# heyoeyo/muggled_dpt

Hardware: AMD Instinct MI355X
Metric: depth-maps/sec @518x518 (504x504 model tensor), Depth-Anything-V2 ViT-L (higher is better)
Workload: dtype bf16; 1 GPU; Depth-Anything-V2 ViT-L (vitl), 518x518 image -> 504x504 tensor, batch 32/GPU, bf16 MFMA operands + fp32 accumulate, mdpt_forward via C ABI; global_batch=32, parallelism=dp1, gemm_tile=0, batch_split=True

## Files before the change

### include/mdpt.h

```cpp
#ifndef MDPT_H
#define MDPT_H

#include <stddef.h>
#include <stdint.h>

#ifdef __cplusplus
extern "C" {
#endif

#define MDPT_ABI_VERSION 6

#define MDPT_PREC_BF16 0
#define MDPT_PREC_BF16X3 1
#define MDPT_PREC_FP16 2
#define MDPT_PREC_FP16X3 3
#define MDPT_PREC_MIXED 4

#define MDPT_CLASS_PATCH 0
#define MDPT_CLASS_QKV 1
#define MDPT_CLASS_ATTN 2
#define MDPT_CLASS_PROJ 3
#define MDPT_CLASS_FC1 4
#define MDPT_CLASS_FC2 5
#define MDPT_CLASS_REASM 6
// ... 203 lines not shown
int mdpt_post_align_metrics(const mdpt_depth_pair* pairs_host, const void* pairs_dev, int32_t P, int32_t pred_dtype, int32_t space, double tmin,
                            double tmax, const void* fit_f64, void* metrics_f64, void* scratch, size_t scratch_bytes, void* stream);
int mdpt_post_align_apply(const mdpt_depth_pair* pairs_host, const void* pairs_dev, int32_t P, int32_t pred_dtype, int32_t space, const void* fit_f64,
                          const int64_t* out_offsets_host, const void* out_offsets_dev, double dmin, double dmax, void* out_f32, void* stream);

typedef struct mdpt_guided_pair { const void* map; int32_t h, w; const void* photo; int64_t pitch; int32_t H, W; void* out; int64_t scratch_off; } mdpt_guided_pair;
int mdpt_post_guided_scratch_bytes(const mdpt_guided_pair* pairs_host, int32_t P, size_t* bytes);
int mdpt_post_guided_upsample(const mdpt_guided_pair* pairs_host, const void* pairs_dev, int32_t P, int32_t map_dtype, int32_t radius, double eps,
                              void* scratch, size_t scratch_bytes, void* coeffs_f64, void* stream);

typedef struct mdpt_texture { const void* bgr; int32_t h, w; } mdpt_texture;
int mdpt_post_render_scratch_bytes(int32_t B, int32_t V, int32_t nv, int32_t nf, int32_t out_h, int32_t out_w, size_t* bytes);
int mdpt_post_render(const void* xyz_f32, const void* uv_f32, const void* faces_i32, const void* counts_i32, int32_t B, int32_t nv, int32_t nf,
                     int32_t mode, const mdpt_texture* tex_host, const void* tex_dev, const void* view_proj_f64, int32_t V, int32_t out_h, int32_t out_w,
                     int32_t cull_back, double point_size, void* color_bgra, void* depth_f32, void* face_id_i32, void* scratch, size_t scratch_bytes,
                     void* stream);

int mdpt_post_fill_scratch_bytes(int32_t N, int32_t H, int32_t W, size_t* bytes);
int mdpt_post_fill_holes(const void* color_bgra, const void* depth_f32, int32_t N, int32_t H, int32_t W, double band, void* out_bgra, void* out_depth_f32,
                         void* scratch, size_t scratch_bytes, void* stream);

int mdpt_post_video_scratch_bytes(int32_t T, int32_t h, int32_t w, int32_t out_h, int32_t out_w, size_t* bytes);
int mdpt_post_video_fit(const void* frames, int32_t dtype, int32_t T, int32_t h, int32_t w, const void* prev_frame, const void* ab_in_f64, const void* started_i32,
                        int32_t rounds, double c, double cut_corr, void* table_f64, void* ab_out_f64, void* sums_f64, void* scratch, size_t scratch_bytes,
                        void* stream);
int mdpt_post_video_filter(const void* frames, int32_t dtype, int32_t T, int32_t h, int32_t w, const void* table_f64, const void* prev_out_f32, double alpha,
                           double tau, void* out_f32, void* stream);
int mdpt_post_video_display(const void* stable_f32, int32_t T, int32_t h, int32_t w, const void* table_f64, const void* range_in_f32, const void* started_i32,
                            int32_t out_h, int32_t out_w, int32_t reverse, const void* cmap_bgr, double range_rate, void* out_bgr, void* ranges_f32,
                            void* range_out_f32, void* scratch, size_t scratch_bytes, void* stream);

#define MDPT_REFOCUS_MAX_RADIUS 32
#define MDPT_REFOCUS_TILE 32
typedef struct mdpt_refocus_pair { const void* map; int32_t h, w; const void* photo; int64_t pitch; int32_t H, W; void* out; int64_t scratch_off, tile_off; } mdpt_refocus_pair;
int mdpt_post_refocus_scratch_bytes(const mdpt_refocus_pair* records_host, int32_t n, int32_t max_radius, size_t* bytes);
int mdpt_post_refocus(const mdpt_refocus_pair* records_host, const void* records_dev, int32_t n, int32_t dtype, int32_t space, double focus,
                      const double* focus_xy, double aperture, double focus_range, int32_t max_radius, void* scratch, size_t scratch_bytes, void* radius_out,
                      void* defocus_out, void* stream);

#define MDPT_NORMALS_MAX_STEP 16
#define MDPT_NORMALS_TILE 32
#define MDPT_NORMALS_MAX_LIGHTS 64
typedef struct mdpt_normals_pair { const void* map; int32_t h, w; const void* photo; int64_t pitch; int32_t H, W; void* normals; void* encoded; void* relit; int64_t scratch_off, tile_off; double kx, ky; int32_t step, pad; } mdpt_normals_pair;
int mdpt_post_normals_scratch_bytes(const mdpt_normals_pair* records_host, int32_t n, size_t* bytes);
int mdpt_post_normals(const mdpt_normals_pair* records_host, const void* records_dev, int32_t n, int32_t dtype, int32_t space, double min_depth,
                      double max_depth, double edge_ratio, const void* lights_dev, int32_t num_lights, double ambient, double diffuse, double specular,
                      int32_t shininess_log2, void* scratch, size_t scratch_bytes, void* stream);

#define MDPT_SHADOWS_MAX_REACH 32
#define MDPT_SHADOWS_AO_DIRECTIONS 8
typedef struct mdpt_shadows_pair { const void* map; int32_t h, w; const void* photo; int64_t pitch; int32_t H, W, gh, gw; void* ao; void* vis; void* relit; int64_t scratch_off, tile_off, gtile_off; double kx, ky; int32_t step, pad; } mdpt_shadows_pair;
int mdpt_post_shadows_scratch_bytes(const mdpt_shadows_pair* records_host, int32_t n, size_t* bytes);
int mdpt_post_shadows(const mdpt_shadows_pair* records_host, const void* records_dev, int32_t n, int32_t dtype, int32_t space, double min_depth,
                      double max_depth, double edge_ratio, const void* lights_dev, int32_t num_lights, double ambient, double diffuse, double specular,
                      int32_t shininess_log2, int32_t shadow_reach, double shadow_bias, double shadow_thickness, int32_t ao_reach, double ao_radius,
                      double ao_bias, double ao_strength, void* scratch, size_t scratch_bytes, void* stream);

#define MDPT_SEGMENT_TILE 32
typedef struct mdpt_segment_image { const void* map; int32_t h, w; void* labels; int64_t scratch_off, region_off, tile_off, pixel_off; } mdpt_segment_image;
typedef struct mdpt_segment_photo { const void* labels; int32_t h, w; const void* photo; int64_t pitch; int32_t H, W; void* bgra; void* mask; int64_t region_off; int32_t regions, pad; } mdpt_segment_photo;
int mdpt_segment_scratch_bytes(const mdpt_segment_image* records_host, int32_t n, size_t* bytes);
int mdpt_segment_depth(const mdpt_segment_image* records_host, const void* records_dev, int32_t n, int32_t dtype, int32_t space, double step,
                       int32_t connectivity, int32_t min_area, void* scratch, size_t scratch_bytes, void* counts, void* area, void* bbox, void* first,
                       void* vrange, void* sum_q, void* range, void* stream);
int mdpt_segment_colors(const mdpt_segment_image* records_host, const void* records_dev, int32_t n, void* colors, void* stream);
int mdpt_segment_cutout(const mdpt_segment_photo* records_host, const void* records_dev, int32_t n, const void* picks_dev, int32_t num_picks,
                        int32_t by_label, void* selected, size_t selected_bytes, int32_t invert, void* stream);

#define MDPT_LOCALFIT_MAX_GRID 256
#define MDPT_LOCALFIT_MAX_RADIUS 64
#define MDPT_LOCALFIT_CHUNK 2048
typedef struct mdpt_localfit_pair { const void* pred; int32_t ph, pw; const void* truth; const void* valid; int32_t H, W, gh, gw; int64_t cell_off, scratch_off; void* out; } mdpt_localfit_pair;
int mdpt_localfit_scratch_bytes(const mdpt_localfit_pair* records_host, int32_t n, size_t* bytes);
int mdpt_localfit_fit(const mdpt_localfit_pair* records_host, const void* records_dev, int32_t n, int32_t pred_dtype, int32_t space, int32_t radius,
                      double prior, double tmin, double tmax, void* moments_f64, void* fit_f64, void* sums_f64, void* coeffs_f64, void* scratch,
                      size_t scratch_bytes, void* stream);
int mdpt_localfit_apply(const mdpt_localfit_pair* records_host, const void* records_dev, int32_t n, int32_t pred_dtype, int32_t space,
                        const void* coeffs_f64, double dmin, double dmax, void* stream);

int mdpt_export_tap(mdpt_handle* h, int32_t which, void* out_f32, void* workspace, size_t workspace_bytes, void* stream);

int mdpt_debug_set_stop(mdpt_handle* h, int32_t block, int32_t step);
int mdpt_debug_set_ksplit_min(mdpt_handle* h, int32_t min_k_tiles, int32_t four_k_tiles);
int mdpt_debug_set_reassemble_overlap(mdpt_handle* h, int32_t on);
int mdpt_debug_set_wscale_policy(mdpt_handle* h, int32_t all);
int mdpt_debug_set_side_stream_priority(mdpt_handle* h, int32_t prio);
int mdpt_debug_set_side_stream_probe(mdpt_handle* h, int32_t on);
int mdpt_debug_side_stream_info(mdpt_handle* h, int32_t* candidates, int32_t* rejected);
int mdpt_debug_read(mdpt_handle* h, const char* name, void* out_f32, size_t out_floats, void* workspace, size_t workspace_bytes,
                    void* stream);

int mdpt_debug_set_operand_format(int32_t fp16);

int mdpt_debug_gemm(const void* a_bf16, const void* w_bf16, void* out_f32, void* out_bf16, int32_t M, int32_t N, int32_t K,
                    int32_t tile, int32_t iters, void* stream, void* dbg_times_or_null);
int mdpt_debug_attention(const void* q_bf16, const void* k_bf16, const void* vt_bf16, void* out_bf16, int32_t B, int32_t heads, int32_t N,
                         int32_t npad, int32_t npadv, int32_t iters, void* stream);
typedef struct mdpt_attn_form {
    const void* q_hi; const void* q_lo; const void* k_hi; const void* k_lo;
    const void* vt_hi; const void* vt_lo;
    void* out_hi; void* out_lo;
    int32_t B, heads, N, npad, npadv, F;
    int32_t x3;
    const float* bias_lut; int32_t bias_elen; const int32_t* tq; const int32_t* tk;
    int32_t head_dim;
    int32_t win_nw; const int32_t* rowmap; const int32_t* region; int32_t region_ld;
    int32_t bias_run4;
    int32_t bias_row;
    int32_t bias_ww;
    const float* swin_ls;
    int32_t out_ld;
    int32_t allow_split_kv;
} mdpt_attn_form;
int mdpt_debug_attention_form(const mdpt_attn_form* form, void* stream);
int mdpt_debug_attn_weights_form(const mdpt_attn_form* form, void* out_f32, void* stream);
int mdpt_debug_conv3(const void* in_bf16, const void* w_packed_bf16, const void* bias_f32, const void* skip_f32, const void* up_f32, int32_t Hu,
                     int32_t Wu, void* out_f32, void* out_bf16, int32_t relu_bf16, int32_t B, int32_t H, int32_t W, int32_t Cin, int32_t Cout,
                     int32_t path, int32_t tile, int32_t iters, void* stream, void* dbg_times, const void* in_lo_bf16_or_null,
                     const void* w_lo_bf16_or_null, void* out_lo_bf16_or_null);
typedef struct mdpt_gemm_form {
    const void* a_hi; const void* a_lo; const void* w_hi; const void* w_lo;
    int32_t M, N, K, lda, ldw, npass;
    int32_t amode, ekind, tile, act;
    int32_t tok_np, tok_stride;
    int32_t Hi, Wi, Cin, Ho, Wo, cstride;
    const void* bias; const void* gamma; const void* resid;
    int32_t ldr, bias_img_stride, bias_img_rows;
    void* out_f32; void* out_hi; void* out_lo;
    int32_t ldc, relu_bf16, acc_init;
    const void* wscale;
    void* q_hi; void* q_lo; void* k_hi; void* k_lo; void* vt_hi; void* vt_lo;
    int32_t F, heads, npad, npadv;
    float qscale;
    const void* pos;
    int32_t d2s_k, d2s_cout;
    const void* head_w; const void* head_b; void* head_out;
    int32_t head_sigmoid, head_out_dtype;
    int32_t ksplit, ks_all;
    void* ks_part;
} mdpt_gemm_form;
int mdpt_debug_gemm_form(const mdpt_gemm_form* form, void* stream);
int mdpt_debug_ksplit_finish(const mdpt_gemm_form* form, void* stream);

int mdpt_profile_enable(int on);
int mdpt_profile_report(char* json_buf, size_t capacity);

int mdpt_set_gemm_tile(mdpt_handle* h, int32_t tile);

int mdpt_allgather(void* comm, const void* send_dev, void* recv_dev, size_t count_per_rank, int32_t dtype, void* stream);

#ifdef __cplusplus
}
#endif
#endif
```

### muggled_dpt_amd/csrc/gemm.hip

```cpp

#include "mdpt_kernels.h"
#include "mdpt_prof.h"
#include "f8_cross.h"
#include <stdio.h>
#include <stdlib.h>

#pragma clang fp contract(off)

namespace {

#include "mfma_common.inc"
#include "gemm_common.inc"
#include "gemm_epilogue_strip.inc"
#include "gemm_lockstep.inc"
#include "gemm8_epilogues.inc"
#include "gemm8.inc"

template <int AMODE, int EKIND, int DMODE, bool F8 = false>
int launch_pp_mode(const GemmParams& p, hipStream_t stream) {
    constexpr unsigned LDS = 2 * 65536;
    if constexpr (MDPT_OP_IS_F16 && !F8 && (EKIND == MDPT_E_GENERIC || EKIND == MDPT_E_D2S) && DMODE != DM_RINIT) {
        if (p.f8) return launch_pp_mode<AMODE, EKIND, DMODE, true>(p, stream);
    }
    constexpr auto kern = gemm8_kernel<AMODE, EKIND, DMODE, F8>;
    if (const int e = mdpt_lds_limit<kern>(LDS)) return e;
    const int tiles = ((p.M + 255) / 256) * ((p.N + 255) / 256);
    const char* prof_name = mdpt_kernel_label<kern>(F8 ? "gemm8_kernel<%d, %d, %d, f8>" : "gemm8_kernel<%d, %d, %d>", AMODE, EKIND, DMODE);
    MdptProfScope prof(prof_name, 2.0 * (p.M_alg > 0 ? p.M_alg : p.M) * p.N * p.K, stream);
    const int ks = (AMODE == MDPT_A_DENSE && EKIND == MDPT_E_GENERIC && DMODE == DM_F32 && p.ksplit > 1) ? p.ksplit : 1;
    hipLaunchKernelGGL(kern, dim3(tiles, ks), dim3(512), LDS, stream, p);
    return (int)hipGetLastError();
}

template <int AMODE, int EKIND>
int launch_pp(const GemmParams& p, hipStream_t stream) {
    if constexpr (EKIND == MDPT_E_GENERIC) {
        const int dmode = generic_direct_mode(p);
        if (dmode == DM_BF16) return launch_pp_mode<AMODE, EKIND, DM_BF16>(p, stream);
        if (dmode == DM_RESID) return launch_pp_mode<AMODE, EKIND, DM_RESID>(p, stream);
        if (dmode == DM_F32) return launch_pp_mode<AMODE, EKIND, DM_F32>(p, stream);
        if constexpr (AMODE == MDPT_A_DENSE) {
            if (dmode == DM_RINIT) return launch_pp_mode<AMODE, EKIND, DM_RINIT>(p, stream);
        }
        return launch_pp_mode<AMODE, EKIND, DM_NONE>(p, stream);
    } else if constexpr (EKIND == MDPT_E_QKV) {
        return launch_pp_mode<AMODE, EKIND, DM_QK>(p, stream);
    } else if constexpr (EKIND == MDPT_E_SWQKV) {
        return launch_pp_mode<AMODE, EKIND, DM_SWQK>(p, stream);
    } else {
        return launch_pp_mode<AMODE, EKIND, DM_NONE>(p, stream);
    }
}

template <int BM, int BN, int WM, int WN, int BK, int NST, int MINW, int AMODE, int EKIND, bool F8 = false>
int launch_cfg(const GemmParams& p, hipStream_t stream) {
    constexpr int LDS = NST * (BM + BN) * BK * 2;
    if constexpr (MDPT_OP_IS_F16 && !F8 && BK == 64 && (EKIND == MDPT_E_GENERIC || EKIND == MDPT_E_D2S) && !(BM == 256 && BN == 256)) {
        if (p.f8) return launch_cfg<BM, BN, WM, WN, BK, NST, MINW, AMODE, EKIND, true>(p, stream);
    }
    constexpr auto kern = gemm_kernel<BM, BN, WM, WN, BK, NST, MINW, AMODE, EKIND, F8>;
    if (const int e = mdpt_lds_limit<kern>(LDS)) return e;
    const int tiles = ((p.M + BM - 1) / BM) * ((p.N + BN - 1) / BN);
    const char* prof_name = mdpt_kernel_label<kern>(F8 ? "gemm_kernel<%d, %d, %d, %d, %d, %d, %d, %d, %d, f8>" : "gemm_kernel<%d, %d, %d, %d, %d, %d, %d, %d, %d>", BM, BN, WM, WN, BK, NST, MINW, AMODE, EKIND);
    MdptProfScope prof(prof_name, 2.0 * (p.M_alg > 0 ? p.M_alg : p.M) * p.N * p.K, stream);
    const int ks = ((AMODE == MDPT_A_DENSE || AMODE == MDPT_A_CONV3) && EKIND == MDPT_E_GENERIC && BM == 64 && BN == 64 && BK == 64 && p.ksplit > 1) ? p.ksplit : 1;
    hipLaunchKernelGGL(kern, dim3(tiles, ks), dim3(64 * WM * WN), LDS, stream, p);
    return (int)hipGetLastError();
}

int resolve_tile(const GemmParams& p) {
    int tile = p.tile;
    if (p.ksplit > 1 && p.ks_all) return MDPT_TILE_64x64;
    if (p.ksplit > 1) {
        const long wgs = (long)((p.M + 255) / 256) * ((p.N + 255) / 256) * p.ksplit;
        const int kt = (p.K / 64 / p.ksplit) * p.npass;
        const bool pp = p.tile == MDPT_TILE_PP256 || (p.tile == MDPT_TILE_AUTO && wgs >= (p.throughput_mode ? 70 : 140));
        return (pp && p.amode == MDPT_A_DENSE && generic_direct_mode(p) == DM_F32 && kt >= 4 && !(kt & 1) && (p.N & 255) == 0) ? MDPT_TILE_PP256 : MDPT_TILE_64x64;
    }
    if (tile == MDPT_TILE_AUTO) {
        const long tiles256 = (long)((p.M + 255) / 256) * ((p.N + 255) / 256);
        const long tiles128 = (long)((p.M + 127) / 128) * ((p.N + 127) / 128);
        const long ncol = (p.N + 255) / 256 * 256;
        const bool cols_ok = (ncol - p.N) * 4 <= ncol;
        const bool big = cols_ok && tiles256 >= (p.throughput_mode ? 70 : 140);
        tile = big ? MDPT_TILE_PP256 : (tiles128 <= 352 ? MDPT_TILE_64x64 : MDPT_TILE_128x128);
        if (!big && tiles128 > 352 && p.N <= 64) return -1;
    }
    if (tile == MDPT_TILE_PP256 && (((p.K / 64) * p.npass) & 1) && !p.f8) tile = (p.K / 64) * p.npass <= 3 && p.tile == MDPT_TILE_AUTO ? MDPT_TILE_64x64 : MDPT_TILE_256x256;
    if (tile == MDPT_TILE_PP256 && p.f8 && ((p.K & 255) || (p.N & 255))) tile = MDPT_TILE_128x128;
    if (tile == MDPT_TILE_256x256 && p.f8) tile = MDPT_TILE_128x128;
    if (tile == MDPT_TILE_PP256 && p.bias_img_stride && p.ekind == MDPT_E_QKV && !(HAVE_IMGB && p.bias_img_rows >= 256)) tile = MDPT_TILE_256x256;
    return tile;
}
template <int AMODE, int EKIND>
int launch_tile(const GemmParams& p, hipStream_t stream) {
    int tile = resolve_tile(p);
    if (tile < 0) return launch_cfg<128, 64, 4, 1, 64, 2, 2, AMODE, EKIND>(p, stream);
    if constexpr (EKIND == MDPT_E_GENERIC) {
        if (tile == MDPT_TILE_PP256 && p.acc_init &&
            !(AMODE == MDPT_A_DENSE && generic_direct_mode(p) == DM_RINIT && (p.K / 64) * p.npass >= 4 && !p.f8))
            tile = MDPT_TILE_256x256;
    }
    if (tile == MDPT_TILE_64x64) {
        if constexpr ((AMODE == MDPT_A_DENSE || AMODE == MDPT_A_CONV3) && EKIND == MDPT_E_GENERIC) {
            if (ktiles_total(p, p.K / (p.ksplit > 1 ? p.ksplit : 1)) >= 32) return launch_cfg<64, 64, 2, 2, 64, 3, 1, AMODE, EKIND>(p, stream);
        }
        return launch_cfg<64, 64, 2, 2, 64, 2, 1, AMODE, EKIND>(p, stream);
    }
    if (tile == MDPT_TILE_PP256) return launch_pp<AMODE, EKIND>(p, stream);
    if (tile == MDPT_TILE_256x128) return launch_cfg<256, 128, 2, 2, 32, 3, 2, AMODE, EKIND>(p, stream);
    if (tile == MDPT_TILE_256x256) return launch_cfg<256, 256, 2, 4, 64, 2, 1, AMODE, EKIND>(p, stream);
    return launch_cfg<128, 128, 2, 2, 64, 2, 1, AMODE, EKIND>(p, stream);
}
// ... 51 lines not shown
```

### muggled_dpt_amd/csrc/gemm8.inc

```
template <int AMODE, bool F8 = false>
struct HalfStager {
    static constexpr int A_BYTES = 256 * 128;
#ifdef MDPT_GEMM8_BUF_STAGING
    static constexpr bool BUFFERED = AMODE != MDPT_A_CONV3;
#else
    static constexpr bool BUFFERED = false;
#endif
    __amdgpu_buffer_rsrc_t rs_a, rs_w;
    unsigned a_voff[4], b_voff;
    int a_soff, b_soff, a_row_step, b_row_step;
    const op_t* a_base_hi; const op_t* a_base_lo; const op_t* w_base_hi; const op_t* w_base_lo;
    size_t a_bytes, w_bytes;
    const op_t* a_ptr[4];
    int a_pix[4], a_y[4], a_x[4], a_ko[4];
    const op_t* b_ptr[4];
    ptrdiff_t a_hi_minus_lo, w_lo_minus_hi;
    const op_t* conv_plane;
    int a_pass, a_k0, a_tap, a_ci, b_pass, b_k0;
    int st_m0, st_n0, b_step;
    bool a_f8, b_f8;

    __device__ __forceinline__ void place_a(const GemmParams& p, int pass, int wave, int lane) {
        const int lrow = lane >> 3;
        a_f8 = pass < p.npass - 1;
// ... 128 lines not shown
                const size_t e = (size_t)(a_pix[i] + iy * p.Wi + ix) * p.Cin + a_ci;
                src = ok ? conv_plane + ((F8 && a_f8) ? (e >> 1) : e) + a_ko[i] : p.zero_page + a_ko[i];
            } else {
                src = a_ptr[i];
                a_ptr[i] += 64;
            }
            glds16(src, buf + (wave + 8 * i) * 1024);
        }
        if (F8 && H == 1 && a_f8) {
            a_k0 += 128;
            if (AMODE == MDPT_A_CONV3) { if (++a_tap == 9) { a_tap = 0; a_ci += 128; } }
            if (a_k0 == p.K) {
                a_k0 = 0; a_tap = 0; a_ci = 0;
                ++a_pass;
                place_a(p, a_pass, wave, threadIdx.x & 63);
            }
        } else
        if (H == 1) {
            a_k0 += 64;
            if (AMODE == MDPT_A_CONV3) {
                if (++a_tap == 9) { a_tap = 0; a_ci += 64; }
            }
            if (a_k0 == p.K) {
                a_k0 = 0; a_tap = 0; a_ci = 0;
                const ptrdiff_t da = (a_pass == 0 ? a_hi_minus_lo : 0) - p.K;
                if (a_pass == 0) conv_plane = p.A_hi;
#pragma unroll
                for (int i = 0; i < 4; ++i)
                    if (AMODE != MDPT_A_CONV3) a_ptr[i] += da;
                ++a_pass;
            }
        }
    }

    template <int H>
    __device__ __forceinline__ void issue_b(const GemmParams& p, char* buf, int wave) {
        typedef __attribute__((address_space(3))) void* lds_ptr_t;
        if constexpr (BUFFERED) {
#pragma unroll
            for (int i = 2 * H; i < 2 * H + 2; ++i)
                __builtin_amdgcn_raw_ptr_buffer_load_lds(rs_w, (lds_ptr_t)(buf + A_BYTES + (wave + 8 * i) * 1024), 16, b_voff, b_soff + i * b_row_step, 0, 0);
            if (H == 1) {
                b_soff += 128;
                if (b_soff == p.K * 2) {
                    b_soff = 0;
                    rs_w = rsrc(b_pass == 0 ? w_base_lo : w_base_hi, w_bytes);
                    ++b_pass;
                }
            }
            return;
        }
        if constexpr (F8) {
#pragma unroll
            for (int i = 2 * H; i < 2 * H + 2; ++i) glds16((const op_t*)((const char*)b_ptr[0] + i * b_step), buf + A_BYTES + (wave + 8 * i) * 1024);
            if (H == 1) b_ptr[0] += 64;
        } else {
#pragma unroll
        for (int i = 2 * H; i < 2 * H + 2; ++i) {
            glds16(b_ptr[i], buf + A_BYTES + (wave + 8 * i) * 1024);
            b_ptr[i] += 64;
        }
        }
        if (F8 && H == 1 && b_f8) {
            b_k0 += 128;
            if (b_k0 == p.K) {
                b_k0 = 0;
                ++b_pass;
                place_b(p, b_pass, wave, threadIdx.x & 63);
            }
        } else
        if (H == 1) {
            b_k0 += 64;
            if (b_k0 == p.K) {
                b_k0 = 0;
                const ptrdiff_t dw = (b_pass == 0 ? w_lo_minus_hi : -w_lo_minus_hi) - p.K;
#pragma unroll
                for (int i = 0; i < 4; ++i) b_ptr[i] += dw;
                ++b_pass;
            }
        }
    }
};

template <int AMODE, int EKIND, bool SW, bool RI = false, bool FAST = false, bool F8 = false>
__device__ __forceinline__ void gemm8_body(const GemmParams& p, char* smem, const int dmode, const int m0, const int n0,
                                           const unsigned long long t_start) {
    static_assert(!RI || SW, "residual-initialised accumulators use the swapped operand order (4 consecutive columns per lane)");
    static_assert(!F8 || (!FAST && !RI && MDPT_HAVE_F8), "fp8 cross terms: state-machine stager, fp16 build");
    static_assert(!FAST || AMODE == MDPT_A_DENSE, "the stateless staging is for dense rows");
    constexpr int A_BYTES = 256 * 128, BUF = 2 * A_BYTES;
    const int tid = threadIdx.x, lane = tid & 63;
    const int wave = __builtin_amdgcn_readfirstlane(tid >> 6);
    const int grp = wave >> 2, wc = wave & 3;
    unsigned long long t_first = 0, t_loop = 0;
    constexpr bool swapped = SW;
    HalfStager<AMODE, F8> st;
    if constexpr (!FAST) st.init(p, m0, n0, wave, lane);
    typedef __attribute__((address_space(3))) void* lds_ptr_t;
    __amdgpu_buffer_rsrc_t rs_a, rs_w;
    unsigned fa_voff = 0, fb_voff = 0;
    int fa_step = 0, fb_step = 0;
    if constexpr (FAST) {
        const int rows_here = p.M - m0 < 256 ? p.M - m0 : 256, cols_here = p.N - n0 < 256 ? p.N - n0 : 256;
        rs_a = tile_rsrc(p.A_hi + (size_t)m0 * p.lda, (size_t)rows_here * p.lda * 2);
        rs_w = tile_rsrc(p.W_hi + (size_t)n0 * p.ldw, ((size_t)(cols_here - 1) * p.ldw + p.K) * 2);
        const int r = wave * 8 + (lane >> 3);
        const int koff = ((lane & 7) ^ ((r >> 1) & 7)) * 8;
        fa_voff = (unsigned)(r * p.lda + koff) * 2u;
        fb_voff = (unsigned)(r * p.ldw + koff) * 2u;
        fa_step = 64 * p.lda * 2;
        fb_step = 64 * p.ldw * 2;
    }
#define ISSUE_A(H_, BUF_, KB_)                                                                                          \
    do {                                                                                                                \
        if constexpr (FAST) {                                                                                           \
            _Pragma("unroll") for (int i = 2 * (H_); i < 2 * (H_) + 2; ++i)                                             \
                __builtin_amdgcn_raw_ptr_buffer_load_lds(rs_a, (lds_ptr_t)((BUF_) + (wave + 8 * i) * 1024), 16, fa_voff, (KB_) + i * fa_step, 0, 0); \
        } else {                                                                                                        \
            st.template issue_a<H_>(p, BUF_, wave);                                                                     \
        }                                                                                                               \
    } while (0)
#define ISSUE_B(H_, BUF_, KB_)                                                                                          \
    do {                                                                                                                \
        if constexpr (FAST) {                                                                                           \
            _Pragma("unroll") for (int i = 2 * (H_); i < 2 * (H_) + 2; ++i)                                             \
                __builtin_amdgcn_raw_ptr_buffer_load_lds(rs_w, (lds_ptr_t)((BUF_) + 256 * 128 + (wave + 8 * i) * 1024), 16, fb_voff, (KB_) + i * fb_step, 0, 0); \
        } else {                                                                                                        \
            st.template issue_b<H_>(p, BUF_, wave);                                                                     \
        }                                                                                                               \
    } while (0)

    const int l15 = lane & 15, lh = lane >> 4, key = (l15 >> 1) & 7;
    const int a_off0 = (grp * 64 + l15) * 128 + ((lh ^ key) << 4), a_off1 = (grp * 64 + l15) * 128 + (((4 + lh) ^ key) << 4);
    const int b_off0 = A_BYTES + (wc * 32 + l15) * 128 + ((lh ^ key) << 4), b_off1 = A_BYTES + (wc * 32 + l15) * 128 + (((4 + lh) ^ key) << 4);

    f32x4 acc[2][2][4][2];
    if constexpr (!RI) {
#pragma unroll
        for (int a = 0; a < 2; ++a)
#pragma unroll
            for (int b = 0; b < 2; ++b)
#pragma unroll
                for (int i = 0; i < 4; ++i)
#pragma unroll
                    for (int j = 0; j < 2; ++j) acc[a][b][i][j] = f32x4{0.0f, 0.0f, 0.0f, 0.0f};
    }

    opx8 fa[4][2], fb0[2][2], fb1[2][2];
#define LOAD_A(QM_, BUF_)                                                                                             \
    do {                                                                                                              \
        _Pragma("unroll") for (int i = 0; i < 4; ++i) {                                                               \
            fa[i][0] = *(const opx8*)(smem + (BUF_) * BUF + (QM_) * 16384 + i * 2048 + a_off0);                      \
            fa[i][1] = *(const opx8*)(smem + (BUF_) * BUF + (QM_) * 16384 + i * 2048 + a_off1);                      \
        }                                                                                                             \
    } while (0)
#define LOAD_B(DST_, QN_, BUF_)                                                                                       \
    do {                                                                                                              \
        _Pragma("unroll") for (int j = 0; j < 2; ++j) {                                                               \
            DST_[j][0] = *(const opx8*)(smem + (BUF_) * BUF + (QN_) * 16384 + j * 2048 + b_off0);                    \
            DST_[j][1] = *(const opx8*)(smem + (BUF_) * BUF + (QN_) * 16384 + j * 2048 + b_off1);                    \
        }                                                                                                             \
    } while (0)
#define MFMA_Q(QM_, QN_, FB_)                                                                                         \
    do {                                                                                                              \
        __builtin_amdgcn_s_setprio(1);                                                                                \
        _Pragma("unroll") for (int kk = 0; kk < 2; ++kk)                                                              \
            _Pragma("unroll") for (int i = 0; i < 4; ++i)                                                             \
                _Pragma("unroll") for (int j = 0; j < 2; ++j)                                                         \
                    acc[QM_][QN_][i][j] = swapped ? MDPT_MFMA_16x16x32(FB_[j][kk], fa[i][kk], acc[QM_][QN_][i][j], 0, 0, 0) \
                                                  : MDPT_MFMA_16x16x32(fa[i][kk], FB_[j][kk], acc[QM_][QN_][i][j], 0, 0, 0); \
        __builtin_amdgcn_s_setprio(0);                                                                                \
    } while (0)
#if MDPT_HAVE_F8
    int wsc = 0, wsc_lo = 0;
    const int asc = F8_A_SCALE;
    if constexpr (F8) {
#pragma unroll
        for (int b4 = 0; b4 < 4; ++b4) {
            int n = n0 + (b4 >> 1) * 128 + wc * 32 + (b4 & 1) * 16 + l15;
            n = n < p.N ? n : p.N - 1;
            wsc |= (int)p.S8[n] << (8 * b4);
            if (p.npass == 3) wsc_lo |= (int)p.S8_lo[n] << (8 * b4);
        }
    }
#define MFMA_Q8_ONE(QM_, QN_, FB_, I_, J_, WS_)                                                                       \
    do {                                                                                                              \
        if constexpr (swapped) f8_mfma16_w_first<2 * (QN_) + (J_)>(acc[QM_][QN_][I_][J_], f8_cat(FB_[J_][0], FB_[J_][1]), f8_cat(fa[I_][0], fa[I_][1]), WS_, asc); \
        else f8_mfma16_a_first<2 * (QN_) + (J_)>(acc[QM_][QN_][I_][J_], f8_cat(fa[I_][0], fa[I_][1]), f8_cat(FB_[J_][0], FB_[J_][1]), asc, WS_); \
    } while (0)
#define MFMA_Q8(QM_, QN_, FB_, WS_)                                                                                   \
    do {                                                                                                              \
        __builtin_amdgcn_s_setprio(1);                                                                                \
        MFMA_Q8_ONE(QM_, QN_, FB_, 0, 0, WS_); MFMA_Q8_ONE(QM_, QN_, FB_, 0, 1, WS_);                                 \
        MFMA_Q8_ONE(QM_, QN_, FB_, 1, 0, WS_); MFMA_Q8_ONE(QM_, QN_, FB_, 1, 1, WS_);                                 \
        MFMA_Q8_ONE(QM_, QN_, FB_, 2, 0, WS_); MFMA_Q8_ONE(QM_, QN_, FB_, 2, 1, WS_);                                 \
        MFMA_Q8_ONE(QM_, QN_, FB_, 3, 0, WS_); MFMA_Q8_ONE(QM_, QN_, FB_, 3, 1, WS_);                                 \
        __builtin_amdgcn_s_setprio(0);                                                                                \
    } while (0)
#endif
#define ACC_READY(QM_, QN_, N_)                                                                                                          \
    asm volatile("s_waitcnt vmcnt(" #N_ ")"                                                                                              \
                 : "+v"(acc[QM_][QN_][0][0]), "+v"(acc[QM_][QN_][0][1]), "+v"(acc[QM_][QN_][1][0]), "+v"(acc[QM_][QN_][1][1]),           \
                   "+v"(acc[QM_][QN_][2][0]), "+v"(acc[QM_][QN_][2][1]), "+v"(acc[QM_][QN_][3][0]), "+v"(acc[QM_][QN_][3][1])            \
                 :                                                                                                                       \
                 : "memory")

    const int T = F8 ? ktiles_total(p, p.K) : (p.K / 64) * p.npass;
    const int T8 = F8 ? ktiles_f8(p, p.K) : 0, T8a = F8 ? p.K / 128 : 0;
    char* const bufE = smem;
    char* const bufO = smem + BUF;
    ISSUE_A(0, bufE, 0);
    ISSUE_B(0, bufE, 0);
    ISSUE_B(1, bufE, 0);
    ISSUE_A(1, bufE, 0);
    if constexpr (RI) {
        constexpr unsigned OOB = 0xFFFFFFF0u;
        typedef __attribute__((ext_vector_type(4))) int i32x4;
        const int rows_here = p.M - m0 < 256 ? p.M - m0 : 256;
        const unsigned long long base = (unsigned long long)(p.resid + (size_t)m0 * p.ldr);
        i32x4 rs;
        rs[0] = __builtin_amdgcn_readfirstlane((int)(unsigned)base);
        rs[1] = __builtin_amdgcn_readfirstlane((int)(unsigned)(base >> 32) & 0xFFFF);
        rs[2] = __builtin_amdgcn_readfirstlane((int)(unsigned)((size_t)rows_here * p.ldr * 4));
        rs[3] = 0x00020000;
        const unsigned row_b = (unsigned)p.ldr * 4u;
        auto load_quadrant = [&](int qm, int qn) {
#pragma unroll
            for (int j = 0; j < 2; ++j) {
                const int nc = n0 + qn * 128 + wc * 32 + j * 16 + 4 * lh;
                const unsigned col = nc < p.N ? (unsigned)nc * 4u : OOB;
#pragma unroll
                for (int i = 0; i < 4; ++i) {
                    const unsigned row = (unsigned)(qm * 128 + grp * 64 + i * 16 + l15) * row_b;
                    const unsigned off = col == OOB ? OOB : row + col;
                    asm volatile("s_nop 4\n\tbuffer_load_dwordx4 %0, %1, %2, 0 offen" : "=v"(acc[qm][qn][i][j]) : "v"(off), "s"(rs) : "memory");
                }
            }
        };
        load_quadrant(0, 0);
        ISSUE_B(0, bufO, 128);
        ISSUE_A(0, bufO, 128);
        ISSUE_B(1, bufO, 128);
        ISSUE_A(1, bufO, 128);
        load_quadrant(0, 1);
        load_quadrant(1, 1);
        load_quadrant(1, 0);
        WAIT_VM(40);
    } else {
        ISSUE_B(0, bufO, 128);
        ISSUE_A(0, bufO, 128);
        ISSUE_B(1, bufO, 128);
        ISSUE_A(1, bufO, 128);
        WAIT_VM(8);
    }
    BAR();
    if (p.dbg_times) t_first = memtime_now();
    if (grp == 1) BAR();


    const float ri_scale = (MDPT_OP_IS_F16 && RI && p.wscale) ? p.wscale[0] : 1.0f;
#define SCALE_Q(QM_, QN_)                                                                                             \
    do {                                                                                                              \
        if (MDPT_OP_IS_F16 && RI && ri_scale != 1.0f) {                                                               \
            _Pragma("unroll") for (int i = 0; i < 4; ++i)                                                             \
                _Pragma("unroll") for (int j = 0; j < 2; ++j) acc[QM_][QN_][i][j] *= ri_scale;                        \
        }                                                                                                             \
    } while (0)
#define GEMM8_ITER(MORE_, FIRST_, MQ)                                                                                       \
    do {                                                                                                              \
        const int kE = t * 128 + 256, kO = kE + 128;         \
                                                                                                              \
        LOAD_B(fb0, 0, 0); PIN(); LOAD_A(0, 0); PIN();                                                                \
        WAIT_LGKM(8); BAR(); WAIT_LGKM(0); PIN();                                                                     \
        if (FIRST_) { ACC_READY(0, 0, 32); SCALE_Q(0, 0); PIN(); }                     \
        MQ(0, 0, fb0); BAR();                                                                                     \
                                                                                                              \
        LOAD_B(fb1, 1, 0); PIN();                                                                                     \
        if (MORE_) ISSUE_B(0, bufE, kE);                                                             \
        BAR(); WAIT_LGKM(0); PIN();                                                                                   \
        if (FIRST_) { ACC_READY(0, 1, 18); SCALE_Q(0, 1); PIN(); }                               \
        MQ(0, 1, fb1); BAR();                                                                                     \
                                                                                                              \
        LOAD_A(1, 0); PIN();                                                                                          \
        if (MORE_) ISSUE_A(0, bufE, kE);                                                             \
        PIN(); WAIT_LGKM(0); BAR(); PIN();                                                                            \
        if (FIRST_) { ACC_READY(1, 1, 12); SCALE_Q(1, 1); PIN(); }                                \
        MQ(1, 1, fb1); BAR();                                                                                     \
                                                                                                              \
        if (MORE_) { ISSUE_B(1, bufE, kE); ISSUE_A(1, bufE, kE); PIN(); WAIT_VM(8); } else { WAIT_VM(0); }                      \
        BAR();                                                                                                        \
        if (FIRST_) { ACC_READY(1, 0, 8); SCALE_Q(1, 0); PIN(); }  \
        MQ(1, 0, fb0); BAR();                                                                                     \
                                                                                                              \
        LOAD_B(fb0, 0, 1); PIN(); LOAD_A(0, 1); PIN();                                                                \
        WAIT_LGKM(8); BAR(); WAIT_LGKM(0); PIN();                                                                     \
        MQ(0, 0, fb0); BAR();                                                                                     \
                                                                                                              \
        LOAD_B(fb1, 1, 1); PIN();                                                                                     \
        if (MORE_) ISSUE_B(0, bufO, kO);                                                             \
        BAR(); WAIT_LGKM(0); PIN();                                                                                   \
        MQ(0, 1, fb1); BAR();                                                                                     \
                                                                                                              \
        LOAD_A(1, 1); PIN();                                                                                          \
        if (MORE_) ISSUE_A(0, bufO, kO);                                                             \
        PIN(); WAIT_LGKM(0); BAR(); PIN();                                                                            \
        MQ(1, 1, fb1); BAR();                                                                                     \
                                                                                                              \
        if (MORE_) { ISSUE_B(1, bufO, kO); ISSUE_A(1, bufO, kO); PIN(); WAIT_VM(8); }                                          \
        BAR();                                                                                                        \
        MQ(1, 0, fb0); BAR();                                                                                     \
    } while (0)
    if constexpr (FAST) {
        int t = 0;
        if constexpr (RI) {
            GEMM8_ITER(true, true, MFMA_Q);
            t = 2;
        }
        for (; t + 2 < T; t += 2) GEMM8_ITER(true, false, MFMA_Q);
        GEMM8_ITER(false, false, MFMA_Q);
    } else {
        int t = 0;
#if MDPT_HAVE_F8
        if constexpr (F8) {
#define MQ8A(QM_, QN_, FB_) MFMA_Q8(QM_, QN_, FB_, wsc)
#define MQ8B(QM_, QN_, FB_) MFMA_Q8(QM_, QN_, FB_, wsc_lo)
            for (; t < T8a; t += 2) GEMM8_ITER(true, false, MQ8A);
            for (; t < T8; t += 2) GEMM8_ITER(true, false, MQ8B);
#undef MQ8A
#undef MQ8B
        }
#endif
        for (; t < T; t += 2) {
            const bool more = t + 2 < T;
            GEMM8_ITER(more, (RI && t == 0), MFMA_Q);
        }
    }
#undef GEMM8_ITER
#undef SCALE_Q
#undef ACC_READY
#undef ISSUE_A
#undef ISSUE_B
    if (grp == 0) BAR();
#undef LOAD_A
#undef LOAD_B
#undef MFMA_Q
#if MDPT_HAVE_F8
#undef MFMA_Q8
#undef MFMA_Q8_ONE
#endif
    if (p.dbg_times) t_loop = memtime_now();
    if constexpr (SW) {
        if (EKIND == MDPT_E_SWQKV) {
            if (dmode == DM_F32) {
                if (HAVE_IMGB && p.bias_img_stride) epilogue_direct<DM_F32, false, MDPT_ACT_NONE, HAVE_IMGB>(p, acc, m0, n0, grp, wc, lane);
                else epilogue_direct<DM_F32, false, MDPT_ACT_NONE>(p, acc, m0, n0, grp, wc, lane);
            } else if (HAVE_IMGB && p.bias_img_stride) {
                if (p.q_lo) epilogue_swin_qk<true, HAVE_IMGB>(p, acc, m0, n0, grp, wc, lane);
                else epilogue_swin_qk<false, HAVE_IMGB>(p, acc, m0, n0, grp, wc, lane);
            } else if (p.q_lo) {
                epilogue_swin_qk<true>(p, acc, m0, n0, grp, wc, lane);
            } else {
                epilogue_swin_qk<false>(p, acc, m0, n0, grp, wc, lane);
            }
        } else if (EKIND == MDPT_E_QKV) {
            if (HAVE_IMGB && p.bias_img_stride) {
                if (p.q_lo) epilogue_direct<DM_QK, true, MDPT_ACT_NONE, HAVE_IMGB>(p, acc, m0, n0, grp, wc, lane);
                else epilogue_direct<DM_QK, false, MDPT_ACT_NONE, HAVE_IMGB>(p, acc, m0, n0, grp, wc, lane);
            } else if (p.q_lo) epilogue_direct<DM_QK, true, MDPT_ACT_NONE>(p, acc, m0, n0, grp, wc, lane);
            else epilogue_direct<DM_QK, false, MDPT_ACT_NONE>(p, acc, m0, n0, grp, wc, lane);
        } else if (HAVE_IMGB && dmode == DM_BF16 && p.bias_img_stride) {
            if (p.act == MDPT_ACT_GELU) {
                if (p.out_lo) epilogue_direct<DM_BF16, true, MDPT_ACT_GELU, HAVE_IMGB>(p, acc, m0, n0, grp, wc, lane);
                else epilogue_direct<DM_BF16, false, MDPT_ACT_GELU, HAVE_IMGB>(p, acc, m0, n0, grp, wc, lane);
            } else {
                if (p.out_lo) epilogue_direct<DM_BF16, true, MDPT_ACT_NONE, HAVE_IMGB>(p, acc, m0, n0, grp, wc, lane);
                else epilogue_direct<DM_BF16, false, MDPT_ACT_NONE, HAVE_IMGB>(p, acc, m0, n0, grp, wc, lane);
            }
        } else if (dmode == DM_BF16) {
            const int sel = (p.out_lo ? 3 : 0) + (p.act == MDPT_ACT_GELU ? 2 : (p.act == MDPT_ACT_RELU || p.relu_bf16) ? 1 : 0);
            switch (sel) {
                case 0: epilogue_direct<DM_BF16, false, MDPT_ACT_NONE>(p, acc, m0, n0, grp, wc, lane); break;
                case 1: epilogue_direct<DM_BF16, false, MDPT_ACT_RELU>(p, acc, m0, n0, grp, wc, lane); break;
                case 2: epilogue_direct<DM_BF16, false, MDPT_ACT_GELU>(p, acc, m0, n0, grp, wc, lane); break;
                case 3: epilogue_direct<DM_BF16, true, MDPT_ACT_NONE>(p, acc, m0, n0, grp, wc, lane); break;
                case 4: epilogue_direct<DM_BF16, true, MDPT_ACT_RELU>(p, acc, m0, n0, grp, wc, lane); break;
                default: epilogue_direct<DM_BF16, true, MDPT_ACT_GELU>(p, acc, m0, n0, grp, wc, lane); break;
            }
        } else if (dmode == DM_F32 || dmode == DM_RINIT) {
            if (HAVE_IMGB && p.bias_img_stride) epilogue_direct<DM_F32, false, MDPT_ACT_NONE, HAVE_IMGB>(p, acc, m0, n0, grp, wc, lane);
            else epilogue_direct<DM_F32, false, MDPT_ACT_NONE>(p, acc, m0, n0, grp, wc, lane);
        } else {
            epilogue_direct<DM_RESID, false, MDPT_ACT_NONE>(p, acc, m0, n0, grp, wc, lane);
        }
        if (p.dbg_times && tid == 0) {
            const unsigned long long t_issued = memtime_now();
            stamp_record(p.dbg_times, t_start, t_first, t_loop, STAMP_HW_ID, t_issued);
        }
        return;
    }
    if ((EKIND == MDPT_E_QKV && dmode == DM_VT) || (EKIND == MDPT_E_SWQKV && dmode == DM_SWVT)) {
        if (EKIND == MDPT_E_SWQKV) {
            if (HAVE_IMGB && p.bias_img_stride) {
                if (p.vt_lo) epilogue_swin_vt<true, HAVE_IMGB>(p, acc, m0, n0, grp, wc, lane);
                else epilogue_swin_vt<false, HAVE_IMGB>(p, acc, m0, n0, grp, wc, lane);
            } else if (p.vt_lo) epilogue_swin_vt<true>(p, acc, m0, n0, grp, wc, lane);
            else epilogue_swin_vt<false>(p, acc, m0, n0, grp, wc, lane);
        } else if (HAVE_IMGB && p.bias_img_stride) {
            if (p.vt_lo) epilogue_direct_vt<true, HAVE_IMGB>(p, acc, m0, n0, grp, wc, lane);
            else epilogue_direct_vt<false, HAVE_IMGB>(p, acc, m0, n0, grp, wc, lane);
        } else if (p.vt_lo) {
            epilogue_direct_vt<true>(p, acc, m0, n0, grp, wc, lane);
        } else {
            epilogue_direct_vt<false>(p, acc, m0, n0, grp, wc, lane);
        }
        if (p.dbg_times && tid == 0) stamp_record(p.dbg_times, t_start, t_first, t_loop, STAMP_NO_ID);
        return;
    }
    __syncthreads();

    float* strip = (float*)smem + wave * (32 * 32);
#pragma unroll
    for (int qm = 0; qm < 2; ++qm)
#pragma unroll
        for (int qn = 0; qn < 2; ++qn)
#pragma unroll
            for (int rb = 0; rb < 2; ++rb) {
#pragma unroll
                for (int ii = 0; ii < 2; ++ii)
#pragma unroll
                    for (int j = 0; j < 2; ++j)
#pragma unroll
                        for (int r = 0; r < 4; ++r) strip[(ii * 16 + 4 * lh + r) * 32 + j * 16 + l15] = acc[qm][qn][rb * 2 + ii][j][r];
                epilogue_block<32, EKIND>(p, strip, lane, m0 + qm * 128 + grp * 64 + rb * 32, n0 + qn * 128 + wc * 32);
            }
    if (p.dbg_times && tid == 0) stamp_record(p.dbg_times, t_start, t_first, t_loop, 4);
}

__host__ __device__ inline int generic_direct_mode(const GemmParams& p) {
    const bool imgb_ok = HAVE_IMGB && p.bias_img_rows >= 256 && p.bias && !p.gamma && !p.relu_bf16 && p.act != MDPT_ACT_RELU;
    const bool plain = !p.up_src && (!p.bias_img_stride || imgb_ok);
    const bool fits = (size_t)256 * p.ldc * 4 < 0xFFFFFFF0ull;
    if (plain && fits && p.out_hi && !p.out_f32 && !p.gamma && !p.resid && !(p.relu_bf16 && p.act != MDPT_ACT_NONE)) return DM_BF16;
    if (plain && fits && !p.bias_img_stride && p.out_f32 && !p.out_hi && p.gamma && p.resid && p.resid == p.out_f32 && p.bias && p.act == MDPT_ACT_NONE && p.ldr == p.ldc)
        return DM_RESID;
    if (plain && fits && p.acc_init && p.out_f32 && !p.out_hi && !p.gamma && p.resid == p.out_f32 && p.ldr == p.ldc && p.act == MDPT_ACT_NONE && !p.relu_bf16)
        return DM_RINIT;
    if (plain && fits && p.out_f32 && !p.out_hi && !p.gamma && !p.resid && p.act == MDPT_ACT_NONE && !p.relu_bf16) return DM_F32;
    return DM_NONE;
}

template <int AMODE, int EKIND, int DMODE, bool F8 = false>
__global__ __launch_bounds__(512, 1) void gemm8_kernel(const GemmParams p) {
    extern __shared__ __attribute__((aligned(16))) char smem[];
    unsigned long long t_start = 0;
    if (p.dbg_times) t_start = memtime_now();
    int m0, n0;
    tile_coords((p.N + 255) / 256, 256, 256, m0, n0);
    if constexpr (EKIND == MDPT_E_SWQKV) {
        const bool fast = p.npass == 1;
        if (n0 >= 2 * p.F && p.swin_vtokmap) {
            if (fast) gemm8_body<AMODE, EKIND, false, false, true>(p, smem, DM_SWVT, m0, n0, t_start);
            else gemm8_body<AMODE, EKIND, false>(p, smem, DM_SWVT, m0, n0, t_start);
        } else {
            const int dm = n0 >= 2 * p.F ? DM_F32 : DM_SWQK;
            if (fast) gemm8_body<AMODE, EKIND, true, false, true>(p, smem, dm, m0, n0, t_start);
            else gemm8_body<AMODE, EKIND, true>(p, smem, dm, m0, n0, t_start);
        }
    } else if (EKIND == MDPT_E_QKV) {
#ifdef MDPT_GEMM8_NO_FAST
        const bool fast = false;
#else
        const bool fast = AMODE == MDPT_A_DENSE && p.npass == 1;
#endif
        if (n0 + 256 <= 2 * p.F && (size_t)p.M * p.F * 2 < 0xFFFFFFF0ull) {
            if constexpr (AMODE == MDPT_A_DENSE) {
                if (fast) gemm8_body<AMODE, EKIND, true, false, true>(p, smem, DM_QK, m0, n0, t_start);
                else gemm8_body<AMODE, EKIND, true>(p, smem, DM_QK, m0, n0, t_start);
            } else {
                gemm8_body<AMODE, EKIND, true>(p, smem, DM_QK, m0, n0, t_start);
            }
        } else if (n0 >= 2 * p.F && n0 + 256 <= p.N && (size_t)(p.M / p.npad) * p.F * p.npadv * 2 < 0xFFFFFFF0ull) {
            if constexpr (AMODE == MDPT_A_DENSE) {
                if (fast) gemm8_body<AMODE, EKIND, false, false, true>(p, smem, DM_VT, m0, n0, t_start);
                else gemm8_body<AMODE, EKIND, false>(p, smem, DM_VT, m0, n0, t_start);
            } else {
                gemm8_body<AMODE, EKIND, false>(p, smem, DM_VT, m0, n0, t_start);
            }
        } else {
            gemm8_body<AMODE, EKIND, false>(p, smem, DM_NONE, m0, n0, t_start);
        }
    } else if constexpr (AMODE == MDPT_A_DENSE && DMODE == DM_F32) {
        if constexpr (F8) {
            gemm8_body<AMODE, EKIND, true, false, false, true>(p, smem, DMODE, m0, n0, t_start);
            return;
        }
        GemmParams q = p;
        if (p.ksplit > 1) {
            const int z = (int)blockIdx.y, ks = p.K / p.ksplit;
            q.K = ks;
            q.A_hi = p.A_hi + z * ks; q.W_hi = p.W_hi + z * ks;
            if (p.npass >= 2) q.A_lo = p.A_lo + z * ks;
            if (p.npass == 3) q.W_lo = p.W_lo + z * ks;
            if (z > 0) { q.bias = nullptr; q.bias_img_stride = 0; q.out_f32 = p.ks_part + (size_t)(z - 1) * p.M * p.ldc; }
        }
        if (q.npass == 1) gemm8_body<AMODE, EKIND, true, false, true>(q, smem, DMODE, m0, n0, t_start);
        else gemm8_body<AMODE, EKIND, true, false, false>(q, smem, DMODE, m0, n0, t_start);
    } else if constexpr (AMODE == MDPT_A_DENSE && DMODE != DM_NONE) {
#ifdef MDPT_GEMM8_NO_FAST
        if (false) {}
#else
        if (p.npass == 1) gemm8_body<AMODE, EKIND, true, DMODE == DM_RINIT, true>(p, smem, DMODE, m0, n0, t_start);
#endif
        else if constexpr (F8) gemm8_body<AMODE, EKIND, true, false, false, true>(p, smem, DMODE, m0, n0, t_start);
        else gemm8_body<AMODE, EKIND, true, DMODE == DM_RINIT, false>(p, smem, DMODE, m0, n0, t_start);
    } else {
        if constexpr (F8) gemm8_body<AMODE, EKIND, DMODE != DM_NONE, false, false, true>(p, smem, DMODE, m0, n0, t_start);
        else gemm8_body<AMODE, EKIND, DMODE != DM_NONE, DMODE == DM_RINIT>(p, smem, DMODE, m0, n0, t_start);
    }
}
```

### muggled_dpt_amd/csrc/gemm8_epilogues.inc

```
constexpr bool HAVE_IMGB = MDPT_OP_IS_F16 != 0;
enum { DM_NONE = 0, DM_BF16 = 1, DM_RESID = 2, DM_QK = 3, DM_VT = 4, DM_F32 = 5, DM_RINIT = 6, DM_SWQK = 7, DM_SWVT = 8 };

__device__ __forceinline__ __amdgpu_buffer_rsrc_t tile_rsrc(const void* base, size_t bytes) {
    return __builtin_amdgcn_make_buffer_rsrc(const_cast<void*>(base), 0, (int)(unsigned)(bytes < 0xFFFFFFF0ull ? bytes : 0xFFFFFFF0ull), 0x00020000);
}

template <int MODE, bool X3, int ACT, bool IMGB = false>
__device__ __forceinline__ void epilogue_direct(const GemmParams& p, f32x4 (&acc)[2][2][4][2], int m0, int n0, int grp, int wc, int lane) {
    constexpr unsigned OOB = 0xFFFFFFF0u;
    const int l15 = lane & 15, lh = lane >> 4;
    const int rows_here = p.M - m0 < 256 ? p.M - m0 : 256;
    int bnd = 1 << 30;
    const float* bias0 = p.bias;
    const float* bias1 = p.bias;
    if (IMGB) {
        const int img0 = m0 / p.bias_img_rows;
        bnd = (img0 + 1) * p.bias_img_rows - m0;
        bias0 = p.bias + (size_t)img0 * p.bias_img_stride;
        bias1 = bnd < rows_here ? bias0 + p.bias_img_stride : bias0;
    }
    auto pick = [&](const f32x4& a, const f32x4& b, bool next) {
        f32x4 r;
#pragma unroll
        for (int e = 0; e < 4; ++e) r[e] = next ? b[e] : a[e];
        return r;
    };

    if (MODE == DM_F32) {
        const __amdgpu_buffer_rsrc_t rs = tile_rsrc(p.out_f32 + (size_t)m0 * p.ldc, (size_t)rows_here * p.ldc * 4);
        const unsigned row_b = (unsigned)p.ldc * 4u;
        const float inv_s = (MDPT_OP_IS_F16 && p.wscale) ? p.wscale[1] : 1.0f;
#pragma unroll
        for (int qn = 0; qn < 2; ++qn) {
            f32x4 bias[2], biasn[2];
            unsigned col_off[2];
#pragma unroll
            for (int j = 0; j < 2; ++j) {
                const int nc = n0 + qn * 128 + wc * 32 + j * 16 + 4 * lh;
                bias[j] = p.bias ? *(const f32x4*)(bias0 + (nc < p.N ? nc : p.N - 4)) : f32x4{0.0f, 0.0f, 0.0f, 0.0f};
                if (IMGB) biasn[j] = *(const f32x4*)(bias1 + (nc < p.N ? nc : p.N - 4));
                col_off[j] = nc < p.N ? (unsigned)nc * 4u : OOB;
            }
#pragma unroll
            for (int qm = 0; qm < 2; ++qm)
#pragma unroll
                for (int i = 0; i < 4; ++i) {
                    const unsigned row = (unsigned)(qm * 128 + grp * 64 + i * 16 + l15) * row_b;
                    const bool next = IMGB && qm * 128 + grp * 64 + i * 16 + l15 >= bnd;
#pragma unroll
                    for (int j = 0; j < 2; ++j) {
                        const f32x4 a = MDPT_OP_IS_F16 ? acc[qm][qn][i][j] * inv_s : acc[qm][qn][i][j];
                        const f32x4 v = a + (IMGB ? pick(bias[j], biasn[j], next) : bias[j]);
                        __builtin_amdgcn_raw_buffer_store_b128(__builtin_bit_cast(u32x4, v), rs, col_off[j] == OOB ? OOB : row + col_off[j], 0, 0);
                    }
                }
        }
        return;
    }
    if (MODE == DM_RESID) {
        const __amdgpu_buffer_rsrc_t rs = tile_rsrc(p.out_f32 + (size_t)m0 * p.ldc, (size_t)rows_here * p.ldc * 4);
        const unsigned row_b = (unsigned)p.ldc * 4u;
        f32x4 bias[2][2], gam[2][2];
        unsigned col_off[2][2];
#pragma unroll
        for (int qn = 0; qn < 2; ++qn)
#pragma unroll
            for (int j = 0; j < 2; ++j) {
                const int nc = n0 + qn * 128 + wc * 32 + j * 16 + 4 * lh;
                const int ncl = nc < p.N ? nc : p.N - 4;
                bias[qn][j] = *(const f32x4*)(p.bias + ncl);
                gam[qn][j] = *(const f32x4*)(p.gamma + ncl);
                col_off[qn][j] = nc < p.N ? (unsigned)nc * 4u : OOB;
            }
        auto row_off = [&](int g, int i) { return (unsigned)((g >> 1) * 128 + grp * 64 + i * 16 + l15) * row_b; };
        u32x4 old[4][4][2];
        f32x4 res[2][4][2];
        auto load_group = [&](int g) {
#pragma unroll
            for (int i = 0; i < 4; ++i)
#pragma unroll
                for (int j = 0; j < 2; ++j) {
                    const unsigned c = col_off[g & 1][j];
                    old[g][i][j] = __builtin_amdgcn_raw_buffer_load_b128(rs, c == OOB ? OOB : row_off(g, i) + c, 0, 0);
                }
        };
        auto value = [&](int g, int i, int j) {
            return (acc[g >> 1][g & 1][i][j] + bias[g & 1][j]) * gam[g & 1][j] + __builtin_bit_cast(f32x4, old[g][i][j]);
        };
        auto store = [&](int g, int i, int j, f32x4 v) {
            const unsigned c = col_off[g & 1][j];
            __builtin_amdgcn_raw_buffer_store_b128(__builtin_bit_cast(u32x4, v), rs, c == OOB ? OOB : row_off(g, i) + c, 0, 0);
        };
        unsigned long long* stamp = p.dbg_times && threadIdx.x == 0 ? p.dbg_times + (size_t)gridDim.x * 6 + (size_t)blockIdx.x * 16 : nullptr;
        if (stamp) stamp[0] = memtime_now();
        load_group(0);
        load_group(1);
        if (p.dbg_times) {
            if (stamp) stamp[1] = memtime_now();
            asm volatile("s_waitcnt vmcnt(0)" ::: "memory");
            if (stamp) stamp[2] = memtime_now();
        }
#pragma unroll
        for (int g = 0; g < 2; ++g)
#pragma unroll
            for (int i = 0; i < 4; ++i)
#pragma unroll
                for (int j = 0; j < 2; ++j) res[g][i][j] = value(g, i, j);
        load_group(2);
        load_group(3);
#pragma unroll
        for (int g = 0; g < 2; ++g)
#pragma unroll
            for (int i = 0; i < 4; ++i)
#pragma unroll
                for (int j = 0; j < 2; ++j) store(g, i, j, res[g][i][j]);
        if (p.dbg_times) {
            if (stamp) stamp[3] = memtime_now();
            asm volatile("s_waitcnt vmcnt(16)" ::: "memory");
            if (stamp) stamp[4] = memtime_now();
        }
#pragma unroll
        for (int g = 2; g < 4; ++g)
#pragma unroll
            for (int i = 0; i < 4; ++i)
#pragma unroll
                for (int j = 0; j < 2; ++j) store(g, i, j, value(g, i, j));
        if (stamp) stamp[5] = memtime_now();
        return;
    }

    __amdgpu_buffer_rsrc_t rs_hi, rs_lo;
    __amdgpu_buffer_rsrc_t rs_lo8 = tile_rsrc(p.out_hi, 0), rs_a8 = rs_lo8;
    if (MODE == DM_BF16) {
        rs_hi = tile_rsrc(p.out_hi + (size_t)m0 * p.ldc, (size_t)rows_here * p.ldc * 2);
        rs_lo = tile_rsrc(X3 ? p.out_lo + (size_t)m0 * p.ldc : p.out_hi, X3 ? (size_t)rows_here * p.ldc * 2 : 0);
        if (MDPT_HAVE_F8 && X3 && p.out_f8) {
            rs_lo8 = tile_rsrc((const unsigned char*)p.out_lo + (size_t)m0 * p.ldc, (size_t)rows_here * p.ldc);
            rs_a8 = tile_rsrc((const unsigned char*)p.out_lo + p.out_f8 + (size_t)m0 * p.ldc, p.out_a8 ? (size_t)rows_here * p.ldc : 0);
        }
    }
    f32x4 bias_q[2][2], biasn_q[2][2], gam_q[2][2];
#pragma unroll
    for (int qn = 0; qn < 2; ++qn)
#pragma unroll
        for (int j = 0; j < 2; ++j) {
            const int ncol = n0 + qn * 128 + wc * 32 + j * 16 + 4 * lh;
            const int nc = ncol < p.N ? ncol : p.N - 4;
            bias_q[qn][j] = p.bias ? *(const f32x4*)(bias0 + nc) : f32x4{0.0f, 0.0f, 0.0f, 0.0f};
            if (IMGB) biasn_q[qn][j] = *(const f32x4*)(bias1 + nc);
            if (MODE == DM_QK && ncol < p.F) gam_q[qn][j] = f32x4{p.qscale, p.qscale, p.qscale, p.qscale};
            else if (MODE == DM_QK) gam_q[qn][j] = f32x4{1.0f, 1.0f, 1.0f, 1.0f};
        }
#pragma unroll
    for (int qn = 0; qn < 2; ++qn) {
        const int nq = n0 + qn * 128 + wc * 32;
        const int n8 = nq + (lh & 1) * 16 + (lh >> 1) * 8;
        const f32x4(&bias)[2] = bias_q[qn];
        const f32x4(&biasn)[2] = biasn_q[qn];
        const f32x4(&gam)[2] = gam_q[qn];
        int qk_h = 0, qk_d = 0;
        if (MODE == DM_QK) {
            const int which = __builtin_amdgcn_readfirstlane(nq >= p.F);
            const int fcol = n8 - which * p.F;
            qk_h = fcol >> 6; qk_d = fcol & 63;
            const size_t plane = (size_t)p.M * p.F * 2;
            rs_hi = tile_rsrc(which ? p.k_hi : p.q_hi, plane);
            rs_lo = tile_rsrc(X3 ? (which ? p.k_lo : p.q_lo) : p.q_hi, X3 ? plane : 0);
        }
        const bool nok = n8 < p.N;
#pragma unroll
        for (int qm = 0; qm < 2; ++qm) {
            const int rfirst = qm * 128 + grp * 64 + l15;
            int qb = 0, qt = 0;
            if (MODE == DM_QK) {
                qb = (m0 + rfirst) / p.npad;
                qt = m0 + rfirst - qb * p.npad;
            }
#pragma unroll
            for (int i = 0; i < 4; ++i) {
                f32x4 v[2];
                const bool next = IMGB && rfirst + 16 * i >= bnd;
#pragma unroll
                for (int j = 0; j < 2; ++j) {
                    v[j] = acc[qm][qn][i][j] + (IMGB ? pick(bias[j], biasn[j], next) : bias[j]);
                    if (MODE == DM_QK) {
                        v[j] *= gam[j];
                    } else if (ACT == MDPT_ACT_GELU) {
#pragma unroll
                        for (int e = 0; e < 4; e += 2) {
                            const gelu_f32x2 g2 = gelu_erf2(gelu_f32x2{v[j][e], v[j][e + 1]});
                            v[j][e] = g2[0];
                            v[j][e + 1] = g2[1];
                        }
                    } else if (ACT == MDPT_ACT_RELU) {
#pragma unroll
                        for (int e = 0; e < 4; ++e) v[j][e] = fmaxf(v[j][e], 0.0f);
                    }
                }
                unsigned hw_[2][2], lw_[2][2];
#pragma unroll
                for (int j = 0; j < 2; ++j)
#pragma unroll
                    for (int w2 = 0; w2 < 2; ++w2) {
                        const f32x2 pp = {v[j][2 * w2], v[j][2 * w2 + 1]};
                        const opx2 hh = to_op2(pp);
                        hw_[j][w2] = __builtin_bit_cast(unsigned, hh);
                        if (X3) {
                            const f32x2 rr = pp - __builtin_convertvector(hh, f32x2);
                            lw_[j][w2] = __builtin_bit_cast(unsigned, to_op2(rr));
                        }
                    }
                unsigned ph[4], pl[4];
#pragma unroll
                for (int w2 = 0; w2 < 2; ++w2) {
                    auto r = __builtin_amdgcn_permlane16_swap(hw_[0][w2], hw_[1][w2], false, false);
                    ph[w2] = r[0];
                    ph[w2 + 2] = r[1];
                    if (X3) {
                        auto rl = __builtin_amdgcn_permlane16_swap(lw_[0][w2], lw_[1][w2], false, false);
                        pl[w2] = rl[0];
                        pl[w2 + 2] = rl[1];
                    }
                }
                unsigned off;
                if (MODE == DM_BF16) {
                    off = ((unsigned)(rfirst + 16 * i) * (unsigned)p.ldc + (unsigned)n8) * 2u;
                    if (!nok) off = OOB;
                } else {
                    off = (unsigned)((((size_t)(qb * p.heads + qk_h) * p.npad + qt) * 64 + qk_d) * 2);
                    if (!nok || m0 + rfirst + 16 * i >= p.M) off = OOB;
                }
                __builtin_amdgcn_raw_buffer_store_b128(u32x4{ph[0], ph[1], ph[2], ph[3]}, rs_hi, off, 0, 0);
#if MDPT_HAVE_F8
                if (X3 && MODE == DM_BF16 && p.out_f8) {
                    float hv[2][4], vv[2][4];
// ... 131 lines not shown
                    auto r = __builtin_amdgcn_permlane16_swap(hw_[0][w2], hw_[1][w2], false, false);
                    ph[w2] = r[0];
                    ph[w2 + 2] = r[1];
                    if (X3) {
                        auto rl = __builtin_amdgcn_permlane16_swap(lw_[0][w2], lw_[1][w2], false, false);
                        pl[w2] = rl[0];
                        pl[w2 + 2] = rl[1];
                    }
                }
                const unsigned off = dst[qm][i] < 0 ? OOB : (unsigned)(((size_t)(dst[qm][i] + hrow) * 32 + d8) * 2);
                __builtin_amdgcn_raw_buffer_store_b128(u32x4{ph[0], ph[1], ph[2], ph[3]}, rs_hi, off, 0, 0);
                if (X3) __builtin_amdgcn_raw_buffer_store_b128(u32x4{pl[0], pl[1], pl[2], pl[3]}, rs_lo, off, 0, 0);
            }
    }
}

template <bool X3, bool IMGB = false>
__device__ __forceinline__ void epilogue_swin_vt(const GemmParams& p, f32x4 (&acc)[2][2][4][2], int m0, int n0, int grp, int wc, int lane) {
    constexpr unsigned OOB = 0xFFFFFFF0u;
    const int l15 = lane & 15, lh = lane >> 4;
    const size_t plane = (size_t)(p.M / p.swin_N) * p.swin_img_velems * 2;
    const __amdgpu_buffer_rsrc_t rs_hi = tile_rsrc(p.vt_hi, plane);
    const __amdgpu_buffer_rsrc_t rs_lo = tile_rsrc(X3 ? p.vt_lo : p.vt_hi, X3 ? plane : 0);
    int bnd = 1 << 30;
    const float* bias0 = p.bias;
    const float* bias1 = p.bias;
    if (IMGB) {
        const int rows_here = p.M - m0 < 256 ? p.M - m0 : 256;
        const int img0 = m0 / p.bias_img_rows;
        bnd = (img0 + 1) * p.bias_img_rows - m0;
        bias0 = p.bias + (size_t)img0 * p.bias_img_stride;
        bias1 = bnd < rows_here ? bias0 + p.bias_img_stride : bias0;
    }
    float bias_q[2][2], biasn_q[2][2];
    int col_q[2][2];
#pragma unroll
    for (int qn = 0; qn < 2; ++qn)
#pragma unroll
        for (int j = 0; j < 2; ++j) {
            const int n = n0 + qn * 128 + wc * 32 + j * 16 + l15;
            bias_q[qn][j] = p.bias ? bias0[n < p.N ? n : p.N - 1] : 0.0f;
            if (IMGB) biasn_q[qn][j] = bias1[n < p.N ? n : p.N - 1];
            col_q[qn][j] = n < p.N ? (n - 2 * p.F) * p.npadv : -1;
        }
    int dst[2][4];
#pragma unroll
    for (int qm = 0; qm < 2; ++qm) {
        const int r0 = m0 + qm * 128 + grp * 64 + 4 * lh;
        int img = r0 / p.swin_N, t = r0 - img * p.swin_N;
#pragma unroll
        for (int i = 0; i < 4; ++i) {
            dst[qm][i] = r0 + 16 * i < p.M ? img * p.swin_img_velems + p.swin_vtokmap[t] : -1;
            t += 16;
            while (t >= p.swin_N) { t -= p.swin_N; ++img; }
        }
    }
#pragma unroll
    for (int qn = 0; qn < 2; ++qn)
#pragma unroll
        for (int qm = 0; qm < 2; ++qm)
#pragma unroll
            for (int i = 0; i < 4; ++i)
#pragma unroll
                for (int j = 0; j < 2; ++j) {
                    const bool next = IMGB && qm * 128 + grp * 64 + 16 * i + 4 * lh >= bnd;
                    const f32x4 v = acc[qm][qn][i][j] + (next ? biasn_q[qn][j] : bias_q[qn][j]);
                    unsigned hw_[2], lw_[2];
#pragma unroll
                    for (int w2 = 0; w2 < 2; ++w2) {
                        const f32x2 pp = {v[2 * w2], v[2 * w2 + 1]};
                        const opx2 hb = to_op2(pp);
                        hw_[w2] = __builtin_bit_cast(unsigned, hb);
                        if (X3) {
                            const f32x2 rr = pp - __builtin_convertvector(hb, f32x2);
                            lw_[w2] = __builtin_bit_cast(unsigned, to_op2(rr));
                        }
                    }
                    const unsigned off = dst[qm][i] < 0 || col_q[qn][j] < 0 ? OOB : (unsigned)(dst[qm][i] + col_q[qn][j]) * 2u;
                    __builtin_amdgcn_raw_buffer_store_b64(u32x2{hw_[0], hw_[1]}, rs_hi, off, 0, 0);
                    if (X3) __builtin_amdgcn_raw_buffer_store_b64(u32x2{lw_[0], lw_[1]}, rs_lo, off, 0, 0);
                }
}

template <bool X3, bool IMGB = false>
__device__ __forceinline__ void epilogue_direct_vt(const GemmParams& p, f32x4 (&acc)[2][2][4][2], int m0, int n0, int grp, int wc, int lane) {
    constexpr unsigned OOB = 0xFFFFFFF0u;
    const int l15 = lane & 15, lh = lane >> 4;
    const size_t plane = (size_t)(p.M / p.npad) * p.F * p.npadv * 2;
    const __amdgpu_buffer_rsrc_t rs_hi = tile_rsrc(p.vt_hi, plane);
    const __amdgpu_buffer_rsrc_t rs_lo = tile_rsrc(X3 ? p.vt_lo : p.vt_hi, X3 ? plane : 0);
    int bnd = 1 << 30;
    const float* bias0 = p.bias;
    const float* bias1 = p.bias;
    if (IMGB) {
        const int rows_here = p.M - m0 < 256 ? p.M - m0 : 256;
        const int img0 = m0 / p.bias_img_rows;
        bnd = (img0 + 1) * p.bias_img_rows - m0;
        bias0 = p.bias + (size_t)img0 * p.bias_img_stride;
        bias1 = bnd < rows_here ? bias0 + p.bias_img_stride : bias0;
    }
    float bias_q[2][2], biasn_q[2][2];
#pragma unroll
    for (int qn = 0; qn < 2; ++qn)
#pragma unroll
        for (int j = 0; j < 2; ++j) {
            const int n = n0 + qn * 128 + wc * 32 + j * 16 + l15;
            bias_q[qn][j] = bias0[n < p.N ? n : p.N - 1];
            if (IMGB) biasn_q[qn][j] = bias1[n < p.N ? n : p.N - 1];
        }
#pragma unroll
    for (int qn = 0; qn < 2; ++qn) {
        const int ncol = n0 + qn * 128 + wc * 32 + (lh & 1) * 16 + l15;
        const int fcol = ncol - 2 * p.F, hh = fcol >> 6, dd = fcol & 63;
        const bool nok = ncol < p.N;
#pragma unroll
        for (int qm = 0; qm < 2; ++qm) {
            const int mfirst = m0 + qm * 128 + grp * 64 + (lh >> 1) * 8;
            int qb = mfirst / p.npad, qt = mfirst - qb * p.npad;
#pragma unroll
            for (int i = 0; i < 4; ++i) {
                unsigned hw_[2][2], lw_[2][2];
#pragma unroll
                for (int j = 0; j < 2; ++j) {
                    const bool next = IMGB && qm * 128 + grp * 64 + 16 * i + 4 * lh >= bnd;
                    const f32x4 v = acc[qm][qn][i][j] + (next ? biasn_q[qn][j] : bias_q[qn][j]);
#pragma unroll
                    for (int w2 = 0; w2 < 2; ++w2) {
                        const f32x2 pp = {v[2 * w2], v[2 * w2 + 1]};
                        const opx2 hb = to_op2(pp);
                        hw_[j][w2] = __builtin_bit_cast(unsigned, hb);
                        if (X3) {
                            const f32x2 rr = pp - __builtin_convertvector(hb, f32x2);
                            lw_[j][w2] = __builtin_bit_cast(unsigned, to_op2(rr));
                        }
                    }
                }
                unsigned ph[4], pl[4];
#pragma unroll
                for (int w2 = 0; w2 < 2; ++w2) {
                    auto r = __builtin_amdgcn_permlane16_swap(hw_[0][w2], hw_[1][w2], false, false);
                    ph[w2] = r[0];
                    ph[w2 + 2] = r[1];
                    if (X3) {
                        auto rl = __builtin_amdgcn_permlane16_swap(lw_[0][w2], lw_[1][w2], false, false);
                        pl[w2] = rl[0];
                        pl[w2 + 2] = rl[1];
                    }
                }
                unsigned off = (unsigned)((((size_t)(qb * p.heads + hh) * 64 + dd) * p.npadv + qt) * 2);
                if (!nok || mfirst + 16 * i >= p.M) off = OOB;
                __builtin_amdgcn_raw_buffer_store_b128(u32x4{ph[0], ph[1], ph[2], ph[3]}, rs_hi, off, 0, 0);
                if (X3) __builtin_amdgcn_raw_buffer_store_b128(u32x4{pl[0], pl[1], pl[2], pl[3]}, rs_lo, off, 0, 0);
                qt += 16;
                while (qt >= p.npad) { qt -= p.npad; ++qb; }
            }
        }
    }
}
```

### muggled_dpt_amd/csrc/gemm_common.inc

```
#define MDPT_GELU_Q0 1.1511051654815674f
#define MDPT_GELU_Q1 0.4592081904411316f
#define MDPT_GELU_Q2 0.052496179938316345f
#define MDPT_GELU_Q3 -0.00706342002376914f
#define MDPT_GELU_Q4 0.00013693643268197775f
#define MDPT_GELU_Q5 0.00018618021567817777f
#define MDPT_GELU_Q6 -3.93776863347739e-05f
#define MDPT_GELU_Q7 2.8349124931992264e-06f
__device__ __forceinline__ float gelu_erf(float v) {
    const float a = fabsf(v);
    float q = MDPT_GELU_Q7;
    q = __builtin_fmaf(q, a, MDPT_GELU_Q6);
    q = __builtin_fmaf(q, a, MDPT_GELU_Q5);
    q = __builtin_fmaf(q, a, MDPT_GELU_Q4);
    q = __builtin_fmaf(q, a, MDPT_GELU_Q3);
    q = __builtin_fmaf(q, a, MDPT_GELU_Q2);
    q = __builtin_fmaf(q, a, MDPT_GELU_Q1);
    q = __builtin_fmaf(q, a, MDPT_GELU_Q0);
    const float erf_abs = 1.0f - __builtin_amdgcn_exp2f(-(q * a));
    const float h = 0.5f * v;
    return __builtin_fmaf(h, copysignf(erf_abs, v), h);
}

typedef f32x2 gelu_f32x2;
__device__ __forceinline__ gelu_f32x2 gelu_erf2(gelu_f32x2 v) {
// ... 101 lines not shown
                const int hw = p.Ho * p.Wo;
                const int b = m / hw, rem = m - b * hw;
                const int y = rem / p.Wo, x = rem - y * p.Wo;
                a_pix[i] = b * p.Hi * p.Wi;
                a_y[i] = y * p.cstride - 1;
                a_x[i] = x * p.cstride - 1;
            }
        }
#pragma unroll
        for (int i = 0; i < CB; ++i) {
            const int r = (wave + NW * i) * RPC + lrow;
            const int koff = (slot ^ ((r / RPB) & (CPR - 1))) * 8;
            int n = n0 + r;
            n = n < p.N ? n : p.N - 1;
            b_ptr[i] = p.W_hi + (size_t)n * p.ldw + koff + kofs;
        }
        a_hi_minus_lo = p.npass >= 2 ? p.A_hi - p.A_lo : 0;
        w_lo_minus_hi = p.npass == 3 ? p.W_lo - p.W_hi : 0;
        conv_plane = A0;
        st_pass = st_k0 = st_sub = 0;
        st_tap0 = AMODE == MDPT_A_CONV3 ? (kofs >> 6) % 9 : 0;
        st_ci0 = AMODE == MDPT_A_CONV3 ? ((kofs >> 6) / 9) * 64 : 0;
        st_tap = st_tap0; st_ci = st_ci0;
        st_m0 = m0; st_n0 = n0; st_f8 = false;
        if constexpr (F8) place(p, 0, wave, lane);
    }

    __device__ __forceinline__ void issue(const GemmParams& p, char* slab_base, int wave) {
        char* sA = slab_base;
        char* sB = slab_base + A_BYTES;
#pragma unroll
        for (int i = 0; i < CA; ++i) {
            const op_t* src;
            if (AMODE == MDPT_A_CONV3) {
                const int ky = (st_tap * 11) >> 5, kx = st_tap - 3 * ky;
                const int iy = a_y[i] + ky, ix = a_x[i] + kx;
                const bool ok = (unsigned)iy < (unsigned)p.Hi && (unsigned)ix < (unsigned)p.Wi;
                const size_t e = (size_t)(a_pix[i] + iy * p.Wi + ix) * p.Cin + st_ci + st_sub;
                src = ok ? conv_plane + ((F8 && st_f8) ? (e >> 1) : e) + a_ko[i] : p.zero_page + a_ko[i];
            } else {
                src = a_ptr[i];
                a_ptr[i] += BK;
            }
            glds16(src, sA + (wave + NW * i) * 1024);
        }
#pragma unroll
        for (int i = 0; i < CB; ++i) {
            glds16(b_ptr[i], sB + (wave + NW * i) * 1024);
            b_ptr[i] += BK;
        }
        if (F8 && st_f8) {
            st_k0 += 128;
            if (AMODE == MDPT_A_CONV3) { if (++st_tap == 9) { st_tap = 0; st_ci += 128; } }
            if (st_k0 == kspan) {
                st_k0 = 0; st_tap = 0; st_ci = 0; st_sub = 0;
                ++st_pass;
                place(p, st_pass, wave, threadIdx.x & 63);
            }
            return;
        }
        st_k0 += BK;
        if (AMODE == MDPT_A_CONV3) {
            st_sub += BK;
            if (st_sub == 64) {
                st_sub = 0;
                if (++st_tap == 9) { st_tap = 0; st_ci += 64; }
            }
        }
        if (st_k0 == kspan) {
            st_k0 = 0; st_tap = st_tap0; st_ci = st_ci0; st_sub = 0;
            const ptrdiff_t da = (st_pass == 0 ? a_hi_minus_lo : 0) - kspan;
            const ptrdiff_t dw = (st_pass == 0 ? w_lo_minus_hi : -w_lo_minus_hi) - kspan;
            if (st_pass == 0) conv_plane = p.A_hi;
#pragma unroll
            for (int i = 0; i < CA; ++i)
                if (AMODE != MDPT_A_CONV3) a_ptr[i] += da;
#pragma unroll
            for (int i = 0; i < CB; ++i) b_ptr[i] += dw;
            ++st_pass;
        }
    }
};

__device__ __forceinline__ void tile_coords(int tiles_n, int BM, int BN, int& m0, int& n0) {
    const int nwg = gridDim.x, swz = xcd_tile();
    if (tiles_n >= 8 && (tiles_n & 3) == 0) {
        const int tiles_m = nwg / tiles_n, per_panel = tiles_m * 4;
        const int panel = swz / per_panel, r = swz - panel * per_panel;
        m0 = (r >> 2) * BM;
        n0 = (panel * 4 + (r & 3)) * BN;
        return;
    }
    m0 = (swz / tiles_n) * BM;
    n0 = (swz % tiles_n) * BN;
}
```

### muggled_dpt_amd/csrc/mdpt_debug.cpp

```cpp
#include "mdpt_internal.h"

extern "C" {

int mdpt_debug_set_stop(mdpt_handle* h, int32_t block, int32_t step) {
    if (!h) return fail(MDPT_E_INVALID, "null handle");
    h->dbg_block = block; h->dbg_step = step;
    return 0;
}

int mdpt_debug_set_reassemble_overlap(mdpt_handle* h, int32_t on) {
    if (!h) return fail(MDPT_E_INVALID, "null handle");
    if (on < 0 || on > 2) return fail(MDPT_E_INVALID, "reassemble overlap: 0 = off, 1 = the library's rule, 2 = always");
    h->overlap_reasm = on;
    return 0;
}

int mdpt_debug_set_wscale_policy(mdpt_handle* h, int32_t all) {
    if (!h) return fail(MDPT_E_INVALID, "null handle");
    h->wscale_all = all ? 1 : 0;
    h->finalized = false;
    return 0;
}

int mdpt_debug_set_side_stream_priority(mdpt_handle* h, int32_t prio) {
    if (!h || prio < -1 || prio > 1) return fail(MDPT_E_INVALID, "null handle or priority class outside -1 .. 1");
    if (h->side_ncand) return fail(MDPT_E_STATE, "the side stream exists already (set the class before the first forward)");
    h->side_prio = prio;
    return 0;
}

int mdpt_debug_set_side_stream_probe(mdpt_handle* h, int32_t on) {
    if (!h) return fail(MDPT_E_INVALID, "null handle");
    if (h->side_ncand) return fail(MDPT_E_STATE, "the side stream exists already (set this before the first forward)");
    h->side_probe = on ? 1 : 0;
    return 0;
}

int mdpt_debug_side_stream_info(mdpt_handle* h, int32_t* candidates, int32_t* rejected) {
    if (!h || !candidates || !rejected) return fail(MDPT_E_INVALID, "null argument");
    *candidates = h->side_ncand;
    *rejected = h->side_rejected;
    return 0;
}

int mdpt_debug_set_ksplit_min(mdpt_handle* h, int32_t min_k_tiles, int32_t four_k_tiles) {
    if (!h || min_k_tiles < 2 || four_k_tiles < 4) return fail(MDPT_E_INVALID, "null handle or thresholds below 2 / 4 K tiles");
    h->ks_min_ktiles = min_k_tiles;
    h->ks_big_ktiles = four_k_tiles;
    return 0;
}

int mdpt_debug_read(mdpt_handle* h, const char* name, void* out_f32, size_t out_floats, void* workspace, size_t workspace_bytes,
                    void* stream) {
    if (!h || !name || !out_f32) return fail(MDPT_E_INVALID, "null argument");
    if (!h->has_last && !h->has_stage_plan) return fail(MDPT_E_STATE, "mdpt_debug_read needs a preceding mdpt_forward");
    if (h->swin) return fail(MDPT_E_UNSUPPORTED, "mdpt_debug_read: internal buffer names are defined for the ViT families only");
    Ctx c;
    c.h = h; c.p = h->has_last ? h->last_plan : h->stage_plan; c.ws = (char*)workspace; c.s = (hipStream_t)stream;
    CHK(check_ws(h, c.p, workspace, workspace_bytes));
    const Plan& p = c.p;
    const size_t rows = (size_t)p.B * p.npad;
    const std::string n = name;
    const size_t* planes = nullptr;
    size_t f32_off = SIZE_MAX, elems = 0;
    size_t bf16_only[3] = {SIZE_MAX, SIZE_MAX, 0};
    const bool bf16_head = head_tail_fused(h) && mdpt_head_tail_scale_ok(8 * p.gh, 8 * p.gw, p.H, p.W);
    const size_t px[4] = {(size_t)16 * p.Np, (size_t)4 * p.Np, (size_t)p.Np, (size_t)p.Np / 4};
    if (n == "im2col") { planes = p.im2col; elems = (size_t)p.B * p.Np * h->Kpatch; }
    else if (n == "pos") { f32_off = p.pos; elems = (size_t)p.Np * h->F; }
    else if (n == "resid") { f32_off = p.resid; elems = rows * h->F; }
    else if (n == "xn") { planes = p.xn; elems = rows * h->F; }
    else if (n == "q") { planes = p.q; elems = (size_t)p.B * h->heads * p.npad * 64; }
    else if (n == "k") { planes = p.k; elems = (size_t)p.B * h->heads * p.npad * 64; }
    else if (n == "vt") { planes = p.vt; elems = (size_t)p.B * h->heads * 64 * p.npadv; }
    else if (n == "att") { planes = p.att; elems = rows * h->F; }
    else if (n == "hbuf") { planes = p.hbuf; elems = rows * 4 * h->F; }
    else if (n == "h1") {
        elems = (size_t)p.B * 64 * p.Np * h->C2p;
        if (bf16_head) { bf16_only[0] = p.h1; if (h->terms(CLS_HEAD_TAIL) == 2) bf16_only[1] = p.h1 + elems * 2; planes = bf16_only; } else { f32_off = p.h1; }
    }
    else if (n == "h1u") {
        if (bf16_head) return fail(MDPT_E_STATE, "h1u does not exist on the fused head-tail path (the upsampled map only ever lives in LDS tiles)");
        planes = p.h1u; elems = (size_t)p.B * p.H * p.W * h->C2p;
    }
    else if (n == "fused") {
        if (head_upsamples_bf16(h))
            CHK(OPLC(mdpt_launch_upsample_bf16, c.at<op_t>(p.flo[0]), c.pl(p.fused).hi, p.B, 4 * p.gh, 4 * p.gw, 8 * p.gh, 8 * p.gw, h->Cp, c.s));
        planes = p.fused; elems = (size_t)p.B * 64 * p.Np * h->Cp;
    }
    else if (n == "u0") { planes = p.u0; elems = (size_t)p.B * px[0] * h->hidp[0]; }
    else if (n == "u1") { planes = p.u1; elems = (size_t)p.B * px[1] * h->hidp[1]; }
    else if (n == "d3") { planes = p.d3; elems = (size_t)p.B * px[3] * h->hidp[3]; }
    else if (n.size() == 2 && n[0] == 't' && n[1] >= '0' && n[1] <= '3') { const int i = n[1] - '0'; planes = p.t[i]; elems = (size_t)p.B * p.Np * h->hidp[i]; }
    else if (n.size() == 4 && n.compare(0, 3, "flo") == 0 && n[3] >= '0' && n[3] <= '3') {
        const int i = n[3] - '0';
        elems = (size_t)p.B * px[i] * h->Cp;
        if (i == 0 && head_upsamples_bf16(h)) { bf16_only[0] = p.flo[0]; planes = bf16_only; } else { f32_off = p.flo[i]; }
    }
    else if (n.size() == 3 && n.compare(0, 2, "xf") == 0 && n[2] >= '0' && n[2] <= '3') { const int i = n[2] - '0'; f32_off = p.x_f32[i]; elems = (size_t)p.B * px[i] * h->Cp; }
    else if (n.size() == 3 && n.compare(0, 2, "a1") == 0 && n[2] >= '0' && n[2] <= '3') { const int i = n[2] - '0'; planes = p.a1[i]; elems = (size_t)p.B * px[i] * h->Cp; }
    else if (n.size() == 3 && n.compare(0, 2, "b2") == 0 && n[2] >= '0' && n[2] <= '3') { const int i = n[2] - '0'; planes = p.b2[i]; elems = (size_t)p.B * px[i] * h->Cp; }
    else return fail(MDPT_E_INVALID, "unknown debug buffer \"%s\"", name);
    if (out_floats < elems) return fail(MDPT_E_WORKSPACE, "debug buffer %s needs %zu floats, got %zu", name, elems, out_floats);
    if (planes) {
        Planes pl = c.pl(planes);
        CHK(OPLC(mdpt_launch_tokens_export, pl.hi, pl.lo, nullptr, (float*)out_f32, 1, (int)(elems / 4), (int)(elems / 4), 4, 0, c.s, pl.lo && planes != bf16_only ? pl.f8 : 0));
    } else {
        CHK(OPLC(mdpt_launch_tokens_export, nullptr, nullptr, c.at<float>(f32_off), (float*)out_f32, 1, (int)(elems / 4), (int)(elems / 4), 4, 0, c.s));
    }
    return 0;
}

int mdpt_debug_gemm(const void* a_bf16, const void* w_bf16, void* out_f32, void* out_bf16, int32_t M, int32_t N, int32_t K,
                    int32_t tile, int32_t iters, void* stream, void* dbg_times) {
    if (!a_bf16 || !w_bf16 || (!out_f32 && !out_bf16)) return fail(MDPT_E_INVALID, "null argument");
    GemmParams g;
    memset(&g, 0, sizeof(g));
    g.A_hi = (const op_t*)a_bf16; g.W_hi = (const op_t*)w_bf16;
    g.M = M; g.N = N; g.K = K; g.lda = K; g.npass = 1;
    g.zero_page = (const op_t*)w_bf16;
    g.amode = MDPT_A_DENSE; g.ekind = MDPT_E_GENERIC; g.tile = tile & 255;
    g.act = (tile >> 8) & 3;
    g.out_f32 = (float*)out_f32; g.out_hi = (op_t*)out_bf16; g.ldc = N; g.ldr = N;
    g.dbg_times = (unsigned long long*)dbg_times;
    if ((tile >> 10) & 1) {
        if (!out_f32 || !out_bf16) return fail(MDPT_E_INVALID, "residual mode needs both output buffers");
        g.bias = (const float*)out_bf16; g.gamma = (const float*)out_bf16 + N; g.resid = (const float*)out_f32; g.out_hi = nullptr;
    }
    if ((tile >> 11) & 1) {
        if (!out_f32 || !out_bf16) return fail(MDPT_E_INVALID, "residual mode needs both output buffers");
        g.bias = (const float*)out_bf16; g.resid = (const float*)out_f32; g.out_hi = nullptr; g.acc_init = 1;
    }
    for (int i = 0; i < iters; ++i) CHK(OPLG(mdpt_launch_gemm, g, (hipStream_t)stream));
    return 0;
}

int mdpt_debug_conv3(const void* in_bf16, const void* w_packed_bf16, const void* bias_f32, const void* skip_f32, const void* up_f32, int32_t Hu,
                     int32_t Wu, void* out_f32, void* out_bf16, int32_t relu_bf16, int32_t B, int32_t H, int32_t W, int32_t Cin, int32_t Cout,
                     int32_t path, int32_t tile, int32_t iters, void* stream, void* dbg_times, const void* in_lo_bf16, const void* w_lo_bf16,
                     void* out_lo_bf16) {
    if (Cout != 256 && Cout != 128) return fail(MDPT_E_INVALID, "Cout must be 256 or 128");
    if (w_lo_bf16 && !in_lo_bf16) return fail(MDPT_E_INVALID, "a lo plane of the weights needs one of the input (three passes); the input alone = two passes");
    if (!in_bf16 || !w_packed_bf16 || (!out_bf16 && !out_f32)) return fail(MDPT_E_INVALID, "null argument");
    static op_t* zero_page = nullptr;
    if (!zero_page) {
        if (hipMalloc((void**)&zero_page, 256) != hipSuccess || hipMemset(zero_page, 0, 256) != hipSuccess) return fail(MDPT_E_STATE, "zero page allocation failed");
    }
    if (path == 2 || path == 3) {
        if (Cout != 128 || !out_bf16 || Hu < 2 || Wu < 2) return fail(MDPT_E_INVALID, "upsampled-input form: 128 output channels, bf16 output");
        if (path == 2) {
            Conv3hParams q;
            memset(&q, 0, sizeof(q));
            q.up_in = (const op_t*)in_bf16; q.Hs = Hu; q.Ws = Wu; q.w = (const op_t*)w_packed_bf16; q.bias = (const float*)bias_f32;
            q.out_bf = (op_t*)out_bf16; q.B = B; q.H = H; q.W = W; q.Cin = Cin; q.Cout = 128;
            q.dbg_times = (unsigned long long*)dbg_times;
            if (!OPLG(mdpt_conv3h_supported, q)) return fail(MDPT_E_UNSUPPORTED, "conv3h does not cover this combination");
            for (int i = 0; i < iters; ++i) CHK(OPLG(mdpt_launch_conv3h, q, (hipStream_t)stream));
            return 0;
        }
        if (!out_lo_bf16) return fail(MDPT_E_INVALID, "path 3 needs a scratch map in out_lo_bf16");
        for (int i = 0; i < iters; ++i) {
            CHK(OPLG(mdpt_launch_upsample_bf16, (const op_t*)in_bf16, (op_t*)out_lo_bf16, B, Hu, Wu, H, W, Cin, (hipStream_t)stream));
            GemmParams g;
            memset(&g, 0, sizeof(g));
            g.A_hi = (const op_t*)out_lo_bf16; g.W_hi = (const op_t*)w_packed_bf16;
            g.M = B * H * W; g.N = 128; g.K = 9 * Cin; g.lda = Cin; g.npass = 1; g.zero_page = zero_page;
            g.amode = MDPT_A_CONV3; g.ekind = MDPT_E_GENERIC; g.tile = tile;
            g.Hi = H; g.Wi = W; g.Cin = Cin; g.Ho = H; g.Wo = W; g.cstride = 1;
            g.bias = (const float*)bias_f32; g.out_hi = (op_t*)out_bf16; g.ldc = 128; g.ldr = 128;
            CHK(OPLG(mdpt_launch_gemm, g, (hipStream_t)stream));
        }
        return 0;
    }
    if (path == 1) {
        Conv3hParams q;
        memset(&q, 0, sizeof(q));
        q.in = (const op_t*)in_bf16; q.w = (const op_t*)w_packed_bf16; q.bias = (const float*)bias_f32; q.skip = (const float*)skip_f32;
        q.in_lo = (const op_t*)in_lo_bf16; q.w_lo = (const op_t*)w_lo_bf16; q.out_bf_lo = (op_t*)out_lo_bf16;
        q.up_src = (const float*)up_f32; q.Hu = Hu; q.Wu = Wu; q.out_f32 = (float*)out_f32; q.out_bf = (op_t*)out_bf16; q.relu_bf = relu_bf16;
        q.B = B; q.H = H; q.W = W; q.Cin = Cin; q.Cout = Cout;
        q.dbg_times = (unsigned long long*)dbg_times;
        if (!OPLG(mdpt_conv3h_supported, q)) return fail(MDPT_E_UNSUPPORTED, "conv3h does not cover this combination");
        for (int i = 0; i < iters; ++i) CHK(OPLG(mdpt_launch_conv3h, q, (hipStream_t)stream));
        return 0;
    }
    GemmParams g;
    memset(&g, 0, sizeof(g));
    g.A_hi = (const op_t*)in_bf16; g.W_hi = (const op_t*)w_packed_bf16; g.A_lo = (const op_t*)in_lo_bf16; g.W_lo = (const op_t*)w_lo_bf16;
    g.M = B * H * W; g.N = Cout; g.K = 9 * Cin; g.lda = Cin; g.npass = in_lo_bf16 ? (w_lo_bf16 ? 3 : 2) : 1;
    g.zero_page = zero_page;
    g.amode = MDPT_A_CONV3; g.ekind = MDPT_E_GENERIC; g.tile = tile;
    g.Hi = H; g.Wi = W; g.Cin = Cin; g.Ho = H; g.Wo = W; g.cstride = 1;
    g.bias = (const float*)bias_f32; g.resid = (const float*)skip_f32; g.ldr = Cout;
    g.up_src = (const float*)up_f32; g.Hu = Hu; g.Wu = Wu;
    g.out_f32 = (float*)out_f32; g.out_hi = (op_t*)out_bf16; g.out_lo = (op_t*)out_lo_bf16; g.relu_bf16 = relu_bf16; g.ldc = Cout;
    g.dbg_times = (unsigned long long*)dbg_times;
    for (int i = 0; i < iters; ++i) CHK(OPLG(mdpt_launch_gemm, g, (hipStream_t)stream));
    return 0;
}

int mdpt_debug_gemm_form(const mdpt_gemm_form* f, void* stream) {
    if (!f || !f->a_hi || !f->w_hi) return fail(MDPT_E_INVALID, "null argument");
    if (f->ekind == MDPT_E_SWQKV) return fail(MDPT_E_UNSUPPORTED, "mdpt_debug_gemm_form: the SwinV2 QKV epilogue is not part of this hook");
    static op_t* zero_page = nullptr;
    if (!zero_page) {
        if (hipMalloc((void**)&zero_page, 256) != hipSuccess || hipMemset(zero_page, 0, 256) != hipSuccess) return fail(MDPT_E_STATE, "zero page allocation failed");
    }
    GemmParams g;
    memset(&g, 0, sizeof(g));
    g.A_hi = (const op_t*)f->a_hi; g.A_lo = (const op_t*)f->a_lo; g.W_hi = (const op_t*)f->w_hi; g.W_lo = (const op_t*)f->w_lo;
    g.M = f->M; g.N = f->N; g.K = f->K; g.lda = f->lda; g.ldw = f->ldw; g.npass = f->npass;
    g.zero_page = zero_page;
    g.amode = f->amode; g.ekind = f->ekind; g.tile = f->tile; g.act = f->act;
    g.tok_np = f->tok_np; g.tok_stride = f->tok_stride;
    g.Hi = f->Hi; g.Wi = f->Wi; g.Cin = f->Cin; g.Ho = f->Ho; g.Wo = f->Wo; g.cstride = f->cstride;
    g.bias = (const float*)f->bias; g.gamma = (const float*)f->gamma; g.resid = (const float*)f->resid; g.ldr = f->ldr;
    g.bias_img_stride = f->bias_img_stride; g.bias_img_rows = f->bias_img_rows;
    g.out_f32 = (float*)f->out_f32; g.out_hi = (op_t*)f->out_hi; g.out_lo = (op_t*)f->out_lo; g.ldc = f->ldc;
    g.relu_bf16 = f->relu_bf16; g.acc_init = f->acc_init; g.wscale = (const float*)f->wscale;
    g.q_hi = (op_t*)f->q_hi; g.q_lo = (op_t*)f->q_lo; g.k_hi = (op_t*)f->k_hi; g.k_lo = (op_t*)f->k_lo; g.vt_hi = (op_t*)f->vt_hi; g.vt_lo = (op_t*)f->vt_lo;
    g.F = f->F; g.heads = f->heads; g.npad = f->npad; g.npadv = f->npadv; g.qscale = f->qscale;
    g.pos = (const float*)f->pos;
    g.d2s_k = f->d2s_k; g.d2s_cout = f->d2s_cout;
    g.head_w = (const float*)f->head_w; g.head_b = (const float*)f->head_b; g.head_sigmoid = f->head_sigmoid; g.head_out = f->head_out;
    g.head_out_dtype = f->head_out_dtype;
    g.ksplit = f->ksplit; g.ks_part = (float*)f->ks_part; g.ks_all = f->ks_all;
    CHK(OPLG(mdpt_launch_gemm, g, (hipStream_t)stream));
    return 0;
}

int mdpt_debug_ksplit_finish(const mdpt_gemm_form* f, void* stream) {
    if (!f || !f->ks_part || (!f->out_f32 && !f->out_hi)) return fail(MDPT_E_INVALID, "null argument");
    CHK(OPLG(mdpt_launch_ksplit_finish, (const float*)f->ks_part, (size_t)f->M * f->ldc, f->ksplit, (const float*)f->bias, (float*)f->out_f32, (op_t*)f->out_hi,
             (op_t*)f->out_lo, f->relu_bf16, f->M, f->N, f->ldc, (hipStream_t)stream, 0, 0));
    return 0;
}

int mdpt_debug_attention(const void* q_bf16, const void* k_bf16, const void* vt_bf16, void* out_bf16, int32_t B, int32_t heads, int32_t N,
                         int32_t npad, int32_t npadv, int32_t iters, void* stream) {
    if (!q_bf16 || !k_bf16 || !vt_bf16 || !out_bf16) return fail(MDPT_E_INVALID, "null argument");
    AttnParams a;
    memset(&a, 0, sizeof(a));
    a.q_hi = (const op_t*)q_bf16; a.k_hi = (const op_t*)k_bf16; a.vt_hi = (const op_t*)vt_bf16; a.out_hi = (op_t*)out_bf16;
    a.B = B; a.heads = heads; a.N = N; a.npad = npad; a.npadv = npadv; a.F = heads * 64;
    for (int i = 0; i < iters; ++i) CHK(OPLG(mdpt_launch_attention, a, (hipStream_t)stream));
    return 0;
}

static AttnParams attn_form_params(const mdpt_attn_form* f) {
    AttnParams a;
    memset(&a, 0, sizeof(a));
    a.q_hi = (const op_t*)f->q_hi; a.q_lo = (const op_t*)f->q_lo; a.k_hi = (const op_t*)f->k_hi; a.k_lo = (const op_t*)f->k_lo;
    a.vt_hi = (const op_t*)f->vt_hi; a.vt_lo = (const op_t*)f->vt_lo; a.out_hi = (op_t*)f->out_hi; a.out_lo = (op_t*)f->out_lo;
    a.B = f->B; a.heads = f->heads; a.N = f->N; a.npad = f->npad; a.npadv = f->npadv; a.F = f->F; a.x3 = f->x3;
    a.bias_lut = f->bias_lut; a.bias_elen = f->bias_elen; a.tq = f->tq; a.tk = f->tk;
    a.head_dim = f->head_dim;
    a.win_nw = f->win_nw; a.rowmap = f->rowmap; a.region = f->region; a.region_ld = f->region_ld;
    a.bias_run4 = f->bias_run4; a.bias_row = f->bias_row; a.bias_ww = f->bias_ww;
    a.swin_ls = f->swin_ls; a.out_ld = f->out_ld; a.allow_split_kv = f->allow_split_kv;
    return a;
}

int mdpt_debug_attention_form(const mdpt_attn_form* f, void* stream) {
    if (!f || !f->q_hi || !f->k_hi || !f->vt_hi || !f->out_hi) return fail(MDPT_E_INVALID, "null argument");
    if (f->x3 && (!f->q_lo || !f->k_lo || !f->vt_lo || !f->out_lo)) return fail(MDPT_E_INVALID, "null argument: x3 takes the lo planes");
    CHK(OPLG(mdpt_launch_attention, attn_form_params(f), (hipStream_t)stream));
    return 0;
}

int mdpt_debug_attn_weights_form(const mdpt_attn_form* f, void* out_f32, void* stream) {
    if (!f || !f->q_hi || !f->k_hi || !out_f32) return fail(MDPT_E_INVALID, "null argument");
    CHK(OPLG(mdpt_launch_attn_weights, attn_form_params(f), (float*)out_f32, (hipStream_t)stream));
    return 0;
}

int mdpt_allgather(void* comm, const void* send_dev, void* recv_dev, size_t count_per_rank, int32_t dtype, void* stream) {
    typedef int (*allgather_fn)(const void*, void*, size_t, int, void*, void*);
    static allgather_fn fn = nullptr;
    if (!fn) {
        void* lib = dlopen("librccl.so", RTLD_NOW | RTLD_GLOBAL);
        if (!lib) lib = dlopen("librccl.so.1", RTLD_NOW | RTLD_GLOBAL);
        if (!lib) return fail(MDPT_E_STATE, "cannot load librccl.so: %s", dlerror());
        fn = (allgather_fn)dlsym(lib, "ncclAllGather");
        if (!fn) return fail(MDPT_E_STATE, "ncclAllGather not found in librccl.so");
    }
    if (!tensor_dtype_ok(dtype)) return fail(MDPT_E_INVALID, "bad dtype %d", dtype);
    const int nccl_type = dtype == MDPT_DTYPE_F32 ? 7 : (dtype == MDPT_DTYPE_BF16 ? 9 : 6);
    const int rc = fn(send_dev, recv_dev, count_per_rank, nccl_type, comm, stream);
    if (rc != 0) return fail(MDPT_E_STATE, "ncclAllGather failed with code %d", rc);
    return 0;
}

}
```

### muggled_dpt_amd/csrc/mdpt_internal.h

```cpp

#pragma once
#include <dlfcn.h>
#include <stdarg.h>
#include <stdio.h>
#include <string.h>

#include <map>
#include <string>
#include <vector>

#include "../../include/mdpt.h"
#include "mdpt_kernels.h"

#undef MDPT_FN
#define MDPT_FN(name) name##_f16
extern "C" {
#include "mdpt_launchers.inc"
}
#undef MDPT_FN
#define MDPT_FN(name) name##_bf16
#define OPL_(f16, fn, ...) ((f16) ? fn##_f16(__VA_ARGS__) : fn##_bf16(__VA_ARGS__))
#define OPLC(fn, ...) OPL_(c.h->f16, fn, __VA_ARGS__)
#define OPLH(fn, ...) OPL_(h->f16, fn, __VA_ARGS__)
#define OPLG(fn, ...) OPL_(g_debug_f16, fn, __VA_ARGS__)
#define mdpt_head_tail_supported mdpt_head_tail_supported_bf16
#define mdpt_head_tail_scale_ok mdpt_head_tail_scale_ok_bf16
#define mdpt_beit_relpos_elen mdpt_beit_relpos_elen_bf16

namespace mdpt {

extern thread_local std::string g_err;
extern int g_debug_f16;

int fail(int code, const char* fmt, ...);

#define CHK(expr)                                                                                                   \
    do {                                                                                                            \
        int e_ = (int)(expr);                                                                                       \
        if (e_ != 0) {                                                                                              \
            if (e_ > 0) return fail(e_, "%s: hip error %d (%s)", #expr, e_, hipGetErrorString((hipError_t)e_));      \
            return e_;                                                                                              \
        }                                                                                                           \
    } while (0)

inline bool tensor_dtype_ok(int dt) { return dt == MDPT_DTYPE_F32 || dt == MDPT_DTYPE_BF16 || dt == MDPT_DTYPE_F16; }
inline bool interp_ok(int interp) { return interp == MDPT_INTERP_BILINEAR || interp == MDPT_INTERP_BICUBIC; }

inline int rup(int v, int m) { return (v + m - 1) / m * m; }
inline size_t rup256(size_t v) { return (v + 255) & ~(size_t)255; }

struct WeightSpec {
    std::string name;
    int ndim;
    int64_t shape[4];
    const void* ptr;
    int dtype;
    size_t numel() const {
        size_t n = 1;
        for (int i = 0; i < ndim; ++i) n *= (size_t)shape[i];
        return n;
    }
};

enum { CLS_PATCH = MDPT_CLASS_PATCH, CLS_QKV = MDPT_CLASS_QKV, CLS_ATTN = MDPT_CLASS_ATTN, CLS_PROJ = MDPT_CLASS_PROJ, CLS_FC1 = MDPT_CLASS_FC1,
       CLS_FC2 = MDPT_CLASS_FC2, CLS_REASM = MDPT_CLASS_REASM, CLS_FUSION = MDPT_CLASS_FUSION, CLS_HEAD = MDPT_CLASS_HEAD,
       CLS_FUSION_IN = MDPT_CLASS_FUSION_IN, CLS_HEAD_TAIL = MDPT_CLASS_HEAD_TAIL, CLS_FUSION_PROJ = MDPT_CLASS_FUSION_PROJ, NCLS = MDPT_NUM_CLASSES };

struct Mat {
    int cls;
    int spec, src_ld, src_col0, row_scale;
    int kind, N, K, Np, Kp, ksz;
    size_t off_hi, off_lo;
    op_t* hi;
    op_t* lo;
    size_t off_scale;
    const float* wscale;
    size_t off_w8, off_wlo8, off_s8;
    const uint8_t* w8; const uint8_t* wlo8; const uint8_t* s8; const uint8_t* slo8;
};

enum VecForm { VEC_COPY, VEC_SCALED, VEC_QV_BIAS, VEC_LOG2E };

struct Vec {
    int form, spec, spec2;
    int n, np;
    size_t off;
    float* ptr;
};

struct MatRef { int i = -1; };
struct VecRef { int i = -1; };

struct BlockRefs {
    VecRef ln1_w, ln1_b, ln2_w, ln2_b;
    MatRef qkv, proj, fc1, fc2;
    VecRef qkv_b, proj_b, fc1_b, fc2_b;
    VecRef relpos_lut;
    VecRef logit_scale, cpb_w1, cpb_b1, cpb_w2;
};
struct RcuRefs { MatRef w; VecRef b; };
struct WeightRefs {
    MatRef patch;
    VecRef patch_b, patch_ln_w, patch_ln_b;
    VecRef cls_token, pos_cls, pos_patch, outnorm_w, outnorm_b;
    std::vector<BlockRefs> blocks;
    struct { MatRef reduction; VecRef norm_w, norm_b; } merge[3];
    struct { MatRef readout_tok, readout_cls, resample0, resample1, fuse_proj; VecRef readout_b, resample0_b, resample1_b; } reasm[4];
    struct { RcuRefs rcu[2][2]; MatRef proj; VecRef proj_b; } fusion[4];
    struct { MatRef conv1, proj0, proj0_kc32; VecRef conv1_b, proj0_b, proj2_w, proj2_b; } head;
};

struct Planes {
    op_t* hi = nullptr;
    op_t* lo = nullptr;
    size_t f8 = 0;
    int f8_a8 = 0;
};

extern const char* const kStageNames[4];
extern const char* const kSwinStageNames[4];
constexpr int kCpbHidden = 512;

struct Plan {
    int B, H, W, gh, gw, Np, N, npad, npadv;
    size_t total;
    size_t im2col[3], pos, resid, xn[3], q[3], k[3], vt[3], att[3], hbuf[3], tap[4][3], tapf32;
    size_t t[4][3], u0[3], u1[3], d3[3];
    size_t r_f32[4], r_bf[4][3];
    size_t a1[4][3], x_f32[4], x_bf[4][3], b1[4][3], b2[4][3], flo[4];
    size_t fused[3], h1, h1u[3], scratch;
    size_t scratch_floats;
    size_t tokr[3], cbuf, relpos_lut, relpos_tq, relpos_tk;
    size_t probe;
    size_t poison;
    size_t wrc_mean, wrc_tab;
    size_t swi;
    size_t kspart;
    struct {
        int g0h, g0w;
        size_t resid[4], x, xn[3], q[3], k[3], vt[3], att[3], hb[3], lut, lut_stride, tq, tk, rowmap[2], region[2], tokmap[2], vtokmap[2];
    } sw;
};

}

using namespace mdpt;

struct mdpt_handle {
    mdpt_config cfg;
    int F, heads, nblocks, bps, P, C, Cp, C2, C2p, Kpatch;
    int hid[4], hidp[4];
    bool swin;
    int Pv;
    int gh_hidden, gh_hidden_p;
    int sH[4], sL[4], swh, sww, spre[4];
    bool f16;
    int np[NCLS];
    bool f8ok[NCLS];
    int terms(int cls) const { return np[cls] >= MDPT_PASSES_2F8 ? np[cls] - 2 : np[cls]; }
    bool f8(int cls) const { return np[cls] >= MDPT_PASSES_2F8 && f8ok[cls]; }
    bool x3c(int cls) const { return terms(cls) == 3 && !f8(cls); }
    bool alo(int cls) const { return terms(cls) >= 2; }
    bool wrc_on;
    int wrc_mask;
    bool wrc(int cls) const { return wrc_on && f16 && np[cls] == 1 && (cls == CLS_QKV || cls == CLS_PROJ || cls == CLS_FC1 || cls == CLS_FC2) && ((wrc_mask >> cls) & 1); }
    int wrc_maxn, wrc_maxk;
    int gemm_tile;
    std::vector<WeightSpec> specs;
    std::map<std::string, int> spec_index;
    std::vector<Mat> mats;
    std::vector<Vec> vecs;
    WeightRefs w;
    size_t packed_total;
    size_t zero_off;
    op_t* zero_page;
    bool finalized;
    Plan last_plan;
    bool has_last;
    Plan stage_plan;
    bool has_stage_plan = false;
    int dbg_block, dbg_step;
    int split_min;
    int nonfinite_prop = 1;
    int wscale_all = 0;
    int latency_mode;
    int side_prio;
    int overlap_reasm;
    int grid_cache;
    uint64_t gen;
    struct CacheSlot { const void* ws; int B, H, W; uint64_t gen; bool valid; } cache_slot[2];
    bool cache_hit(const void* ws, int B, int H, int W) const {
        if (!grid_cache) return false;
        for (const CacheSlot& s : cache_slot)
            if (s.valid && s.ws == ws && s.B == B && s.H == H && s.W == W && s.gen == gen) return true;
        return false;
    }
    void cache_store(int slot, const void* ws, int B, int H, int W) { cache_slot[slot] = CacheSlot{ws, B, H, W, gen, true}; }
    void cache_clear() { cache_slot[0].valid = cache_slot[1].valid = false; }
    int ks_min_ktiles, ks_big_ktiles;
    hipStream_t side_stream, side_cand[4], side_for[4];
    int side_pick[4], side_nfor;
    int side_unresolved;
    int side_ncand, side_rejected;
    int side_probe;
    hipEvent_t ev_fork, ev_join;
    ~mdpt_handle() {
        for (int i = 0; i < side_ncand; ++i) hipStreamDestroy(side_cand[i]);
        if (ev_fork) hipEventDestroy(ev_fork);
        if (ev_join) hipEventDestroy(ev_join);
    }

    int add_spec(const std::string& name, std::initializer_list<int64_t> shape) {
        WeightSpec s;
        s.name = name;
        s.ndim = (int)shape.size();
        int i = 0;
        for (int64_t d : shape) s.shape[i++] = d;
        for (; i < 4; ++i) s.shape[i] = 1;
        s.ptr = nullptr;
        s.dtype = MDPT_DTYPE_F32;
        spec_index[name] = (int)specs.size();
        specs.push_back(s);
        return (int)specs.size() - 1;
    }
    MatRef add_mat(int spec, int cls, int kind, int N, int K, int Np, int Kp, int ksz, int src_ld = 0, int src_col0 = 0) {
        Mat m;
        m.spec = spec; m.src_ld = src_ld; m.src_col0 = src_col0; m.row_scale = -1;
        m.cls = cls; m.kind = kind; m.N = N; m.K = K; m.Np = Np; m.Kp = Kp; m.ksz = ksz;
        m.off_hi = packed_total;
        packed_total += rup256((size_t)Np * Kp * 2);
        m.off_lo = SIZE_MAX;
        if (x3c(m.cls) || wrc(m.cls)) {
            if (wrc(m.cls)) { if (Np > wrc_maxn) wrc_maxn = Np; if (Kp > wrc_maxk) wrc_maxk = Kp; } m.off_lo = packed_total; packed_total += rup256((size_t)Np * Kp * 2); }
        m.hi = m.lo = nullptr;
        m.off_scale = SIZE_MAX; m.wscale = nullptr;
        m.off_w8 = m.off_wlo8 = m.off_s8 = SIZE_MAX;
        m.w8 = m.wlo8 = m.s8 = m.slo8 = nullptr;
        if (f8(m.cls) && kind != MDPT_PACK_CONV3_KC32) {
            m.off_w8 = packed_total; packed_total += rup256((size_t)Np * Kp);
            if (terms(m.cls) == 3) { m.off_wlo8 = packed_total; packed_total += rup256((size_t)Np * Kp); }
            m.off_s8 = packed_total; packed_total += rup256((size_t)Np * 2);
        }
        mats.push_back(m);
        return MatRef{(int)mats.size() - 1};
    }
    VecRef add_vec(int spec, int n, int np, int form = VEC_COPY, int spec2 = -1) {
        Vec v;
        v.form = form; v.spec = spec; v.spec2 = spec2; v.n = n; v.np = np;
        v.off = packed_total;
        packed_total += rup256((size_t)np * 4);
        v.ptr = nullptr;
        vecs.push_back(v);
        return VecRef{(int)vecs.size() - 1};
    }
    const Mat& M(MatRef r) const { return mats[r.i]; }
    const float* V(VecRef r) const { return vecs[r.i].ptr; }
};

namespace mdpt {

struct Bump {
    size_t off = 0;
    size_t take(size_t bytes) {
        const size_t o = off;
        off += rup256(bytes);
        return o;
    }
};

struct Ctx {
    const mdpt_handle* h;
    Plan p;
    char* ws;
    hipStream_t s;
    bool split = false;
    hipStream_t tap_stream = nullptr;
    hipEvent_t tap_event = nullptr;
    bool side = false;
    bool a1_done = false;
    unsigned* poison = nullptr;
    bool consts_cached = false;
// ... 80 lines not shown
```

### muggled_dpt_amd/csrc/mdpt_inventory.cpp

```cpp
#include "mdpt_internal.h"

namespace mdpt {

thread_local std::string g_err = "";
int g_debug_f16 = 0;

int fail(int code, const char* fmt, ...) {
    char buf[1024];
    va_list ap;
    va_start(ap, fmt);
    vsnprintf(buf, sizeof(buf), fmt, ap);
    va_end(ap);
    g_err = buf;
    return code;
}

const char* const kStageNames[4] = {"spatial_upx4", "spatial_upx2", "spatial_noscale", "spatial_downx2"};
const char* const kSwinStageNames[4] = {"spatial_noscale", "spatial_downx2", "spatial_downx4", "spatial_downx8"};

static std::string blk_name(const mdpt_handle* h, int block) {
    char buf[96];
    if (h->cfg.family == MDPT_FAMILY_DAV1) snprintf(buf, sizeof(buf), "imgencoder.blocks.%d", block);
    else snprintf(buf, sizeof(buf), "imgencoder.stages.%d.blocks.%d", block / h->bps, block % h->bps);
    return buf;
}
static const char* rcu_seq(const mdpt_handle* h) { return is_midas(h) ? "conv_seq" : "resconv_seq"; }
static const char* proj_seq(const mdpt_handle* h) { return is_midas(h) ? "proj_seq" : "scale_proj_seq"; }

void compute_f8ok(mdpt_handle* h) {
    for (int i = 0; i < NCLS; ++i) h->f8ok[i] = false;
    const bool base = h->f16 && !h->swin;
    const bool cp = base && h->Cp % 128 == 0;
    bool re = base && h->F % 128 == 0;
    for (int i = 0; i < 4; ++i) re = re && h->hidp[i] % 128 == 0;
    h->f8ok[CLS_REASM] = re;
    h->f8ok[CLS_FUSION] = h->f8ok[CLS_FUSION_IN] = h->f8ok[CLS_FUSION_PROJ] = h->f8ok[CLS_HEAD] = cp;
}

static void build_inventory_swin_encoder(mdpt_handle* h);
static void build_inventory_decoder(mdpt_handle* h);
static int check_weight_refs(const mdpt_handle* h);

int build_inventory(mdpt_handle* h) {
    const int F = h->F, P = h->P;
    const int G = h->cfg.base_patch_grid_h * h->cfg.base_patch_grid_w;
    h->specs.clear(); h->spec_index.clear(); h->mats.clear(); h->vecs.clear();
    h->w = WeightRefs();
    WeightRefs& w = h->w;
    h->packed_total = 0;
    h->wrc_maxn = h->wrc_maxk = 0;
    h->zero_off = 0;
    h->packed_total += 256;
    compute_f8ok(h);

    const int s_patch = h->add_spec("patch_embed.proj.weight", {F, 3, P, P});
    const int s_patch_b = h->add_spec("patch_embed.proj.bias", {F});
    w.patch = h->add_mat(s_patch, CLS_PATCH, MDPT_PACK_LINEAR, F, 3 * P * P, F, h->Kpatch, 0);
    w.patch_b = h->add_vec(s_patch_b, F, F);
    if (h->swin) {
        build_inventory_swin_encoder(h);
        build_inventory_decoder(h);
        return check_weight_refs(h);
    }

    const bool beit = is_beit(h);
    const int nlut = (2 * h->cfg.base_patch_grid_h - 1) * (2 * h->cfg.base_patch_grid_w - 1) + 3;
    w.cls_token = h->add_vec(h->add_spec("imgencoder.cls_token", {1, 1, F}), F, F);
    if (!beit) {
        const int s_cls = h->add_spec("imgencoder.posenc.cls_embedding", {1, 1, F});
        const int s_pos = h->add_spec("imgencoder.posenc.base_patch_embedding", {1, G, F});
        const int s_onw = h->add_spec("imgencoder.outnorm.weight", {F});
        const int s_onb = h->add_spec("imgencoder.outnorm.bias", {F});
        w.pos_cls = h->add_vec(s_cls, F, F);
        w.pos_patch = h->add_vec(s_pos, G * F, G * F);
        w.outnorm_w = h->add_vec(s_onw, F, F);
        w.outnorm_b = h->add_vec(s_onb, F, F);
    }

    auto fold_layer_scale = [h](MatRef m, int s_gamma) {
        Mat& mm = h->mats[m.i];
        mm.row_scale = s_gamma;
#ifndef MDPT_NO_WSCALE
        if (h->f16) {
            mm.off_scale = h->packed_total;
            h->packed_total += 256;
        }
#endif
    };
// ... 251 lines not shown
```

### muggled_dpt_amd/csrc/mdpt_kernels.h

```cpp
#pragma once
#include <hip/hip_runtime.h>
#include <stddef.h>
#include <stdint.h>

#include "op_types.h"

enum { MDPT_DT_F32 = 0, MDPT_DT_BF16 = 1, MDPT_DT_F16 = 2 };

enum { MDPT_A_DENSE = 0, MDPT_A_TOKENS = 1, MDPT_A_CONV3 = 2 };
enum { MDPT_E_GENERIC = 0, MDPT_E_QKV = 1, MDPT_E_PATCH = 2, MDPT_E_D2S = 3, MDPT_E_HEAD = 4, MDPT_E_SWQKV = 5 };
enum { MDPT_ACT_NONE = 0, MDPT_ACT_RELU = 1, MDPT_ACT_GELU = 2 };
enum { MDPT_TILE_AUTO = 0, MDPT_TILE_128x128 = 1, MDPT_TILE_256x256 = 2, MDPT_TILE_128x32 = 3, MDPT_TILE_256x128 = 4, MDPT_TILE_PP256 = 5, MDPT_TILE_64x64 = 6 };

struct GemmParams {
    const op_t* A_hi; const op_t* A_lo;
    const op_t* W_hi; const op_t* W_lo;
    int M, N, K;
    int ldw;
    int M_alg;
    int lda;
    int npass;
    const op_t* zero_page;
    int amode, ekind, tile;
    int tok_np, tok_stride;
    int Hi, Wi, Cin, Ho, Wo, cstride;
    const float* bias; const float* gamma; const float* resid; int ldr;
    int bias_img_stride, bias_img_rows;
    const float* up_src; int Hu, Wu;
    int act;
    float* out_f32; op_t* out_hi; op_t* out_lo; int ldc;
    int relu_bf16;
    int acc_init;
    const float* wscale;
    op_t* q_hi; op_t* q_lo; op_t* k_hi; op_t* k_lo; op_t* vt_hi; op_t* vt_lo;
    int F, heads, npad, npadv; float qscale;
    const int* swin_tokmap; const float* swin_logit_scale; int swin_N, swin_img_rows;
    const int* swin_vtokmap; int swin_img_velems;
    const float* pos;
    int d2s_k, d2s_cout;
    const float* head_w; const float* head_b; int head_sigmoid; void* head_out; int head_out_dtype;
    int throughput_mode;
    int f8; size_t a8_off;
    const unsigned char* W8; const unsigned char* W8_lo;
    const unsigned char* S8; const unsigned char* S8_lo;
    size_t out_f8; int out_a8;
    int ksplit; float* ks_part;
    int ks_all;
    unsigned long long* dbg_times;
};


struct Conv3hParams {
    const op_t* in;
    const op_t* up_in; int Hs, Ws;
    const op_t* in_lo;
    const op_t* w;
    const op_t* w_lo;
    const float* bias;
    const float* skip;
    const float* up_src; int Hu, Wu;
    float* out_f32;
    op_t* out_bf;
    op_t* out_bf_lo;
    int relu_bf;
    int B, H, W, Cin;
    int Cout;
    int f8; size_t a8_off;
    const unsigned char* w8; const unsigned char* w8_lo; const unsigned char* s8; const unsigned char* s8_lo;
    size_t out_f8; int out_a8;
    unsigned long long* dbg_times;
};

struct AttnParams {
    const op_t* q_hi; const op_t* q_lo; const op_t* k_hi; const op_t* k_lo;
    const op_t* vt_hi; const op_t* vt_lo;
    op_t* out_hi; op_t* out_lo;
    int B, heads, N, npad, npadv, F;
    int x3;
    const float* bias_lut; int bias_elen; const int* tq; const int* tk;
    int head_dim;
    int win_nw; const int* rowmap; const int* region; int region_ld;
    int bias_run4;
    int bias_row;
    int bias_ww;
    const float* swin_ls;
    int out_ld;
    int allow_split_kv;
    int tail_last;
};

enum { MDPT_PACK_LINEAR = 0,
       MDPT_PACK_CONV3 = 1,
       MDPT_PACK_CONVT = 2,
       MDPT_PACK_CONV3_KC32 = 3 };
struct BeitRelposBatch {
    const float* ref[32]; float* ext0; size_t ext_stride;
    int* tq; int* tk;
    int n, heads, Gh, Gw, gh, gw, N, ntok_pad;
};

struct HeadTailParams {
    const op_t* src;
    const op_t* src_lo;
    const op_t* w_kc;
    const float* bias;
    const float* head_w;
    const float* head_b;
    void* out; int out_dtype;
    int sigmoid;
    int B, Hi, Wi, Ho, Wo;
    unsigned long long* dbg_times;
};

#define MDPT_BGR_RUNS 64
struct BgrRun { const unsigned char* ptr; long long pitch, frame_stride; int ih, iw, count; };
struct BgrRunTable { BgrRun run[MDPT_BGR_RUNS]; int n; };
static_assert(sizeof(BgrRunTable) <= 3072, "BgrRunTable must leave room for the other kernel arguments below HIP's 4 KB limit");

#define MDPT_POST_RUNS 32
struct PostRun { const void* in; size_t off; int ih, iw, oh, ow, count; };
struct PostRunTable { PostRun run[MDPT_POST_RUNS]; int n; };

inline PostRunTable uniform_table(const void* in, int B, int ih, int iw, int oh, int ow) {
// ... 258 lines not shown
```

### muggled_dpt_amd/csrc/mdpt_stages.cpp

```cpp
#include "mdpt_internal.h"

namespace mdpt {

GemmParams base_params(const Ctx& c, const Mat& w, Planes a, int M, int lda) {
    GemmParams g;
    memset(&g, 0, sizeof(g));
    g.npass = c.h->terms(w.cls);
    g.A_hi = a.hi; g.A_lo = g.npass >= 2 ? a.lo : nullptr;
    g.W_hi = w.hi; g.W_lo = g.npass == 3 ? w.lo : nullptr;
    if (g.npass >= 2 && c.h->f8(w.cls) && a.f8 && w.w8) {
        g.f8 = 1; g.a8_off = a.f8;
        g.W8 = w.w8; g.W8_lo = w.wlo8; g.S8 = w.s8; g.S8_lo = w.slo8;
    }
    g.wscale = w.wscale;
    g.M = M; g.N = w.Np; g.K = w.Kp; g.lda = lda;
    g.zero_page = c.h->zero_page;
    g.amode = MDPT_A_DENSE; g.ekind = MDPT_E_GENERIC; g.tile = c.h->gemm_tile;
    g.throughput_mode = c.split ? 1 : 0;
    g.ldc = w.Np; g.ldr = w.Np;
    return g;
}

static void out_planes(GemmParams& g, const Planes& o) {
    g.out_hi = o.hi; g.out_lo = o.lo;
    g.out_f8 = o.lo ? o.f8 : 0; g.out_a8 = o.f8_a8;
}

void as_conv(GemmParams& g, int Hi, int Wi, int Cin, int Ho, int Wo, int stride) {
    g.amode = MDPT_A_CONV3;
    g.Hi = Hi; g.Wi = Wi; g.Cin = Cin; g.Ho = Ho; g.Wo = Wo; g.cstride = stride;
}


int run_pos(const Ctx& c) {
    const mdpt_handle* h = c.h;
    return OPLC(mdpt_launch_posembed, h->V(h->w.pos_patch), c.at<float>(c.p.pos), h->cfg.base_patch_grid_h,
                                h->cfg.base_patch_grid_w, c.p.gh, c.p.gw, h->F, c.s);
}

int run_patchify(const Ctx& c, const void* image, int image_dtype, const Planes& im, int H, int W) {
    const mdpt_handle* h = c.h;
    if (c.bgr.active()) {
        const int runs = c.bgr.table() ? c.p.B : 1;
        const size_t frame_elems = (size_t)(H / h->P) * (W / h->P) * h->Kpatch;
        BgrRunTable t{};
        for (int b0 = 0; b0 < runs; b0 += MDPT_BGR_RUNS) {
            t.n = runs - b0 < MDPT_BGR_RUNS ? runs - b0 : MDPT_BGR_RUNS;
            for (int r = 0; r < t.n; ++r) t.run[r] = c.bgr.run_of(b0 + r, c.p.B);
            CHK(OPLC(mdpt_launch_prepare_patchify, t, c.bgr.round_dtype, im.hi + frame_elems * b0, im.lo ? im.lo + frame_elems * b0 : nullptr, H, W, h->P,
                     h->Kpatch, c.bgr.mean, c.bgr.inv_std, c.bgr.interp, c.s));
        }
        return 0;
    }
    return OPLC(mdpt_launch_patchify, image, image_dtype, im.hi, im.lo, c.p.B, H, W, h->P, h->Kpatch, c.s, c.poison);
}

int run_patch_embed_fused(const Ctx& c, const void* image, int image_dtype) {
    const mdpt_handle* h = c.h;
    const Plan& p = c.p;
    Planes im = c.pl(p.im2col);
    CHK(run_patchify(c, image, image_dtype, im, p.H, p.W));
    const bool beit = is_beit(h);
    if (!beit && !c.consts_cached) CHK(run_pos(c));
    CHK(OPLC(mdpt_launch_init_tokens, c.at<float>(p.resid), h->V(h->w.cls_token), beit ? nullptr : h->V(h->w.pos_cls),
                                p.B, p.N, p.npad, h->F, c.s));
    GemmParams g = base_params(c, h->M(h->w.patch), im, p.B * p.Np, h->Kpatch);
    g.ekind = MDPT_E_PATCH;
    g.bias = h->V(h->w.patch_b);
    g.pos = beit ? nullptr : c.at<float>(p.pos);
    g.out_f32 = c.at<float>(p.resid);
    g.tok_np = p.Np; g.npad = p.npad; g.ldc = h->F;
    CHK(OPLC(mdpt_launch_gemm, g, c.s));
    return 0;
}

int wrc_bias(const Ctx& c, GemmParams& g, const Mat& w, const float* bias, int rows_per_img, int nreal) {
    const mdpt_handle* h = c.h;
    if (!h->wrc(w.cls) || !w.lo) return 0;
    const Plan& p = c.p;
    if (rows_per_img <= 0) { rows_per_img = p.npad; nreal = p.N; }
    op_t* mean = c.at<op_t>(p.wrc_mean);
    float* tab = c.at<float>(p.wrc_tab);
    const int step = nreal >= 1024 ? 8 : (nreal >= 256 ? 4 : 1);
    CHK(OPLC(mdpt_launch_colmean, g.A_hi, g.lda, p.B, rows_per_img, nreal, step, w.Kp, mean, c.s));
    CHK(OPLC(mdpt_launch_wrc_table, mean, w.lo, bias, tab, p.B, w.Np, w.Kp, c.s, w.wscale));
    g.bias = tab; g.bias_img_stride = w.Np; g.bias_img_rows = rows_per_img;
    return 0;
}

bool fc2_ksplit_fits(int rows, int F) { return (long)((rows + 127) / 128) * ((F + 127) / 128) <= 330; }
constexpr int KS_MAX_PARTS = 3;

int run_encoder(const Ctx& c, void* const taps_f32[4]) {
    const mdpt_handle* h = c.h;
    const Plan& p = c.p;
    const int F = h->F, rows = p.B * p.npad;
    float* resid = c.at<float>(p.resid);
    Planes xn = c.pl(p.xn), q = c.pl(p.q), k = c.pl(p.k), vt = c.pl(p.vt), att = c.pl(p.att), hb = c.pl(p.hbuf);
    if (!c.consts_cached) CHK(OPLC(mdpt_launch_zero_vt_pad, vt.hi, vt.lo, p.B * h->heads * 64, p.N, p.npadv, c.s));
    if (att.lo && !h->x3c(CLS_ATTN) && !c.consts_cached) CHK(hipMemsetAsync(att.lo, 0, (size_t)rows * F * 2, c.s));
    const Planes xn_qkv = {xn.hi, h->alo(CLS_QKV) ? xn.lo : nullptr}, xn_fc1 = {xn.hi, h->alo(CLS_FC1) ? xn.lo : nullptr};
// ... 413 lines not shown
```

### muggled_dpt_amd/csrc/mfma_common.inc

```

typedef __attribute__((ext_vector_type(2))) float f32x2;
typedef __attribute__((ext_vector_type(4))) float f32x4;
typedef __attribute__((ext_vector_type(16))) float f32x16;
typedef __attribute__((ext_vector_type(2))) unsigned u32x2;
typedef __attribute__((ext_vector_type(4))) unsigned u32x4;

__device__ __forceinline__ void glds16(const void* gsrc, char* lds_wave_base) {
    __builtin_amdgcn_global_load_lds((const __attribute__((address_space(1))) void*)gsrc,
                                     (__attribute__((address_space(3))) void*)lds_wave_base, 16, 0, 0);
}

__device__ __forceinline__ unsigned long long memtime_now() {
    unsigned long long t;
    asm volatile("s_memtime %0\n\ts_waitcnt lgkmcnt(0)" : "=s"(t)::"memory");
    return t;
}

__device__ __forceinline__ __amdgpu_buffer_rsrc_t plane_rsrc(const void* base, size_t bytes) {
    return __builtin_amdgcn_make_buffer_rsrc(const_cast<void*>(base), 0, (int)(unsigned)(bytes < 0xFFFFFFF0ull ? bytes : 0xFFFFFFF0ull), 0x00020000);
}

#define PIN() __builtin_amdgcn_sched_barrier(0)
#define BAR() do { PIN(); __builtin_amdgcn_s_barrier(); PIN(); } while (0)
#define WAIT_LGKM(N_) asm volatile("s_waitcnt lgkmcnt(" #N_ ")" ::: "memory")
#define WAIT_VM(N_) asm volatile("s_waitcnt vmcnt(" #N_ ")" ::: "memory")
#define WAIT_VM_IMM(N_) asm volatile("s_waitcnt vmcnt(%0)" ::"n"(N_) : "memory")

__device__ __forceinline__ int xcd_tile() {
    const int nwg = gridDim.x, bid = blockIdx.x;
    const int xq = nwg >> 3, xr = nwg & 7, xcd = bid & 7;
    return (xcd < xr ? xcd * (xq + 1) : xr * (xq + 1) + (xcd - xr) * xq) + (bid >> 3);
}

constexpr int STAMP_HW_ID = -1, STAMP_NO_ID = -2;
__device__ __forceinline__ void stamp_record(unsigned long long* dbg_times, unsigned long long t_start, unsigned long long t_first, unsigned long long t_loop,
                                             int xcc_slot, unsigned long long t_issued = 0) {
    asm volatile("s_waitcnt vmcnt(0)" ::: "memory");
    unsigned long long* d = dbg_times + (size_t)blockIdx.x * 6;
    d[0] = t_start; d[1] = t_first; d[2] = t_loop; d[3] = memtime_now();
    if (xcc_slot == STAMP_NO_ID) { d[4] = d[3]; d[5] = 0; return; }
    d[4] = xcc_slot == 4 ? __builtin_amdgcn_s_getreg(20 << 0 | 0 << 6 | 3 << 11) : t_issued;
    d[5] = xcc_slot == 5 ? __builtin_amdgcn_s_getreg(20 << 0 | 0 << 6 | 3 << 11) : __builtin_amdgcn_s_getreg(4 << 0 | 0 << 6 | 31 << 11);
}
```

### muggled_dpt_amd/native.py

```python

from __future__ import annotations

import ctypes
import os
import shutil
import subprocess
from concurrent.futures import ThreadPoolExecutor

CSRC = os.path.join(os.path.dirname(os.path.abspath(__file__)), "csrc")
REPO = os.path.dirname(os.path.dirname(os.path.abspath(__file__)))
LIB_PATH = os.path.join(CSRC, "libmdpt.so")
OPERAND_SOURCES = ("gemm.hip", "conv3h.hip", "attention.hip", "elementwise.hip", "swin.hip", "head.hip")
PLAIN_SOURCES = ("postprocess.hip", "stream_probe.hip", "mdpt_api.cpp", "mdpt_post.cpp", "mdpt_post_geometry.cpp", "mdpt_post_fit.cpp", "mdpt_post_photo.cpp",
                 "mdpt_segment.cpp", "mdpt_localfit.cpp", "mdpt_inventory.cpp", "mdpt_stages.cpp", "mdpt_debug.cpp", "mdpt_prof.cpp")
SOURCES = OPERAND_SOURCES + PLAIN_SOURCES
HEADERS = tuple(sorted(f for f in os.listdir(CSRC) if f.endswith((".h", ".inc")))) + (os.path.join(REPO, "include", "mdpt.h"),)
UNITS = tuple((s, (), os.path.splitext(s)[0]) for s in SOURCES) + tuple((s, ("-DMDPT_OP_F16",), os.path.splitext(s)[0] + "_f16")
                                                                        for s in OPERAND_SOURCES)

ABI_VERSION = 6
DTYPE_F32, DTYPE_BF16, DTYPE_F16 = 0, 1, 2
PREC_BF16 = 0
PREC_BF16X3 = 1
PREC_FP16 = 2
# ... 200 lines not shown
    "mdpt_prepare_image": (ctypes.c_int, [_VP, _I, _I, _VP, _I, _I, _I, ctypes.POINTER(ctypes.c_float), ctypes.POINTER(ctypes.c_float), _I, _VP]),
    "mdpt_forward_bgr": (ctypes.c_int, [_VP, _VP, _I, _I, _I, _I, _I, ctypes.POINTER(ctypes.c_float), ctypes.POINTER(ctypes.c_float), _I, _VP, _I, _VP, _SZ, _VP]),
    "mdpt_forward_bgr_batch": (ctypes.c_int, [_VP, _VP, _I, _I, _I, _I, _I, _I, ctypes.POINTER(ctypes.c_float), ctypes.POINTER(ctypes.c_float), _I, _VP, _I, _VP, _SZ,
                                              _VP]),
    "mdpt_forward_bgr_frames": (ctypes.c_int, [_VP, _VP, _VP, _I, _I, _I, _I, ctypes.POINTER(ctypes.c_float), ctypes.POINTER(ctypes.c_float), _I, _VP, _I, _VP,
                                               _SZ, _VP]),
    "mdpt_prepare_image_region": (ctypes.c_int, [_VP, _I, _I, ctypes.c_int64, _VP, _VP, _I, _I, _I, ctypes.POINTER(ctypes.c_float), ctypes.POINTER(ctypes.c_float), _I,
                                                 _VP]),
    "mdpt_forward_bgr_pitched": (ctypes.c_int, [_VP, _VP, _I, _I, _I, ctypes.c_int64, ctypes.c_int64, _I, _I, _I, ctypes.POINTER(ctypes.c_float),
                                                ctypes.POINTER(ctypes.c_float), _I, _VP, _I, _VP, _SZ, _VP]),
    "mdpt_forward_bgr_regions": (ctypes.c_int, [_VP, _VP, _VP, _VP, _VP, _I, _I, _I, _I, ctypes.POINTER(ctypes.c_float), ctypes.POINTER(ctypes.c_float), _I, _VP, _I,
                                                _VP, _SZ, _VP]),
    "mdpt_post_minmax": (ctypes.c_int, [_VP, _SZ, _VP, _VP, _VP]),
    "mdpt_post_scale_prediction": (ctypes.c_int, [_VP, _I, _I, _I, _VP, _I, _I, _VP, _VP, _VP]),
    "mdpt_post_normalize": (ctypes.c_int, [_VP, _SZ, _VP, _VP, _I, _I, _VP]),
    "mdpt_post_minmax_seg": (ctypes.c_int, [_VP, _I, _I, _I, _I, _VP, _I, _I, _VP, _VP, _VP]),
    "mdpt_post_u8_hist_seg": (ctypes.c_int, [_VP, _I, _I, _SZ, _VP, _I, _VP, _VP, _VP]),
    "mdpt_post_histogram": (ctypes.c_int, [_VP, _I, _SZ, _VP, _VP]),
    "mdpt_post_equalize_lut": (ctypes.c_int, [_VP, _I, _VP, _I, _I, _VP, _VP]),
    "mdpt_post_colorize": (ctypes.c_int, [_VP, _I, _SZ, _VP, _VP, _I, _VP, _VP]),
    "mdpt_post_minmax_images": (ctypes.c_int, [_VP, _VP, _I, _I, _VP, _VP, _VP, _VP, _VP]),
    "mdpt_post_u8_hist_images": (ctypes.c_int, [_VP, _VP, _I, _I, _VP, _I, _VP, _VP, _VP]),
    "mdpt_post_colorize_images": (ctypes.c_int, [_VP, _VP, _I, _VP, _VP, _I, _VP, _VP]),
    "mdpt_post_display_prep": (ctypes.c_int, [_VP, _I, _I, _I, _I, _VP, _I, _I, _VP, _VP, _VP]),
    "mdpt_post_plane_fit": (ctypes.c_int, [_VP, _I, _I, _I, _I, _VP, _VP, _I, _I, _VP, _VP]),
    "mdpt_post_plane_eval": (ctypes.c_int, [_VP, _I, _I, _I, _VP, _VP]),
    "mdpt_post_plane_minmax": (ctypes.c_int, [_VP, _I, _I, _I, _I, _VP, _VP, _D, _VP, _VP]),
    "mdpt_post_threshold": (ctypes.c_int, [_VP, _I, _I, _I, _I, _VP, _VP, _D, _VP, _D, _D, _I, _I, _VP, _VP, _VP]),
    "mdpt_post_edge_mag": (ctypes.c_int, [_VP, _I, _I, _I, _VP, _VP, _I, _VP, _VP, _VP]),
    "mdpt_post_edge_mask": (ctypes.c_int, [_VP, _VP, _I, _SZ, _VP, _VP]),
    "mdpt_post_pack_u24_alpha": (ctypes.c_int, [_VP, _I, _SZ, _VP, _I, _VP, _VP, _VP, _I, _VP, _VP]),
    "mdpt_post_mask_display": (ctypes.c_int, [_VP, _I, _I, _I, _I, _VP, _VP, _D, _VP, _D, _D, _I, _VP, _I, _I, _VP, _VP, _VP]),
    "mdpt_post_mask_cutout_images": (ctypes.c_int, [_VP, _VP, _I, _VP, _VP, _VP, _D, _VP, _VP, _VP, _I, _D, _D, _I, _VP, _VP, _VP]),
    "mdpt_post_block_norm_tiles": (ctypes.c_int, [_VP, _VP, _I, _I, _I, _I, _VP, _VP, _VP]),
    "mdpt_post_mesh_grid": (ctypes.c_int, [_I, _I, _D, ctypes.POINTER(_I), ctypes.POINTER(_I)]),
    "mdpt_post_mesh_scratch_bytes": (ctypes.c_int, [_I, _I, _I, ctypes.POINTER(_SZ)]),
    "mdpt_post_mesh": (ctypes.c_int, [_VP, _I, _I, _I, _I, _I, _VP, _D, _D, _D, _D, _D, _D, _I, _I, _VP, _VP, _VP, _VP, _VP, _VP, _SZ, _VP]),
    "mdpt_post_tile_scratch_bytes": (ctypes.c_int, [_VP, _I, ctypes.POINTER(_SZ)]),
    "mdpt_post_tile_fit": (ctypes.c_int, [_VP, _VP, _I, _I, _VP, _I, _I, _I, _I, _I, _VP, _VP, _VP, _SZ, _VP]),
    "mdpt_post_tile_blend": (ctypes.c_int, [_VP, _VP, _I, _I, _I, _I, _VP, _VP, _D, _VP, _VP]),
    "mdpt_post_align_scratch_bytes": (ctypes.c_int, [_VP, _I, ctypes.POINTER(_SZ)]),
    "mdpt_post_align_fit": (ctypes.c_int, [_VP, _VP, _I, _I, _I, _I, _D, _D, _VP, _VP, _VP, _SZ, _VP]),
    "mdpt_post_align_metrics": (ctypes.c_int, [_VP, _VP, _I, _I, _I, _D, _D, _VP, _VP, _VP, _SZ, _VP]),
    "mdpt_post_align_apply": (ctypes.c_int, [_VP, _VP, _I, _I, _I, _VP, _VP, _VP, _D, _D, _VP, _VP]),
    "mdpt_post_guided_scratch_bytes": (ctypes.c_int, [_VP, _I, ctypes.POINTER(_SZ)]),
    "mdpt_post_guided_upsample": (ctypes.c_int, [_VP, _VP, _I, _I, _I, _D, _VP, _SZ, _VP, _VP]),
    "mdpt_post_render_scratch_bytes": (ctypes.c_int, [_I, _I, _I, _I, _I, _I, ctypes.POINTER(_SZ)]),
    "mdpt_post_render": (ctypes.c_int, [_VP, _VP, _VP, _VP, _I, _I, _I, _I, _VP, _VP, _VP, _I, _I, _I, _I, _D, _VP, _VP, _VP, _VP, _SZ, _VP]),
    "mdpt_post_fill_scratch_bytes": (ctypes.c_int, [_I, _I, _I, ctypes.POINTER(_SZ)]),
    "mdpt_post_fill_holes": (ctypes.c_int, [_VP, _VP, _I, _I, _I, _D, _VP, _VP, _VP, _SZ, _VP]),
    "mdpt_post_video_scratch_bytes": (ctypes.c_int, [_I, _I, _I, _I, _I, ctypes.POINTER(_SZ)]),
    "mdpt_post_video_fit": (ctypes.c_int, [_VP, _I, _I, _I, _I, _VP, _VP, _VP, _I, _D, _D, _VP, _VP, _VP, _VP, _SZ, _VP]),
    "mdpt_post_video_filter": (ctypes.c_int, [_VP, _I, _I, _I, _I, _VP, _VP, _D, _D, _VP, _VP]),
    "mdpt_post_video_display": (ctypes.c_int, [_VP, _I, _I, _I, _VP, _VP, _VP, _I, _I, _I, _VP, _D, _VP, _VP, _VP, _VP, _SZ, _VP]),
    "mdpt_post_refocus_scratch_bytes": (ctypes.c_int, [_VP, _I, _I, ctypes.POINTER(_SZ)]),
    "mdpt_post_refocus": (ctypes.c_int, [_VP, _VP, _I, _I, _I, _D, ctypes.POINTER(_D), _D, _D, _I, _VP, _SZ, _VP, _VP, _VP]),
    "mdpt_post_normals_scratch_bytes": (ctypes.c_int, [_VP, _I, ctypes.POINTER(_SZ)]),
    "mdpt_post_normals": (ctypes.c_int, [_VP, _VP, _I, _I, _I, _D, _D, _D, _VP, _I, _D, _D, _D, _I, _VP, _SZ, _VP]),
    "mdpt_post_shadows_scratch_bytes": (ctypes.c_int, [_VP, _I, ctypes.POINTER(_SZ)]),
    "mdpt_post_shadows": (ctypes.c_int, [_VP, _VP, _I, _I, _I, _D, _D, _D, _VP, _I, _D, _D, _D, _I, _I, _D, _D, _I, _D, _D, _D, _VP, _SZ, _VP]),
    "mdpt_segment_scratch_bytes": (ctypes.c_int, [_VP, _I, ctypes.POINTER(_SZ)]),
    "mdpt_segment_depth": (ctypes.c_int, [_VP, _VP, _I, _I, _I, _D, _I, _I, _VP, _SZ, _VP, _VP, _VP, _VP, _VP, _VP, _VP, _VP]),
    "mdpt_segment_colors": (ctypes.c_int, [_VP, _VP, _I, _VP, _VP]),
    "mdpt_segment_cutout": (ctypes.c_int, [_VP, _VP, _I, _VP, _I, _I, _VP, _SZ, _I, _VP]),
    "mdpt_localfit_scratch_bytes": (ctypes.c_int, [_VP, _I, ctypes.POINTER(_SZ)]),
    "mdpt_localfit_fit": (ctypes.c_int, [_VP, _VP, _I, _I, _I, _I, _D, _D, _D, _VP, _VP, _VP, _VP, _VP, _SZ, _VP]),
    "mdpt_localfit_apply": (ctypes.c_int, [_VP, _VP, _I, _I, _I, _VP, _D, _D, _VP]),
    "mdpt_export_tap": (ctypes.c_int, [_VP, _I, _VP, _VP, _SZ, _VP]),
    "mdpt_set_gemm_tile": (ctypes.c_int, [_VP, _I]),
    "mdpt_set_batch_split": (ctypes.c_int, [_VP, _I]),
    "mdpt_set_latency_mode": (ctypes.c_int, [_VP, _I]),
    "mdpt_set_nonfinite_propagation": (ctypes.c_int, [_VP, _I]),
    "mdpt_debug_gemm": (ctypes.c_int, [_VP, _VP, _VP, _VP, _I, _I, _I, _I, _I, _VP, _VP]),
    "mdpt_debug_attention": (ctypes.c_int, [_VP, _VP, _VP, _VP, _I, _I, _I, _I, _I, _I, _VP]),
    "mdpt_debug_conv3": (ctypes.c_int, [_VP, _VP, _VP, _VP, _VP, _I, _I, _VP, _VP, _I, _I, _I, _I, _I, _I, _I, _I, _I, _VP, _VP, _VP, _VP, _VP]),
    "mdpt_debug_gemm_form": (ctypes.c_int, [ctypes.POINTER(MdptGemmForm), _VP]),
    "mdpt_debug_ksplit_finish": (ctypes.c_int, [ctypes.POINTER(MdptGemmForm), _VP]),
    "mdpt_debug_attention_form": (ctypes.c_int, [ctypes.POINTER(MdptAttnForm), _VP]),
    "mdpt_debug_attn_weights_form": (ctypes.c_int, [ctypes.POINTER(MdptAttnForm), _VP, _VP]),
    "mdpt_profile_enable": (ctypes.c_int, [ctypes.c_int]),
    "mdpt_profile_report": (ctypes.c_int, [ctypes.c_char_p, _SZ]),
    "mdpt_debug_set_stop": (ctypes.c_int, [_VP, _I, _I]),
    "mdpt_debug_set_ksplit_min": (ctypes.c_int, [_VP, _I, _I]),
    "mdpt_debug_set_reassemble_overlap": (ctypes.c_int, [_VP, _I]),
    "mdpt_debug_set_wscale_policy": (ctypes.c_int, [_VP, _I]),
    "mdpt_debug_set_side_stream_priority": (ctypes.c_int, [_VP, _I]),
    "mdpt_debug_set_side_stream_probe": (ctypes.c_int, [_VP, _I]),
    "mdpt_debug_side_stream_info": (ctypes.c_int, [_VP, ctypes.POINTER(ctypes.c_int32), ctypes.POINTER(ctypes.c_int32)]),
    "mdpt_debug_set_operand_format": (ctypes.c_int, [_I]),
    "mdpt_set_grid_cache": (ctypes.c_int, [_VP, _I]),
    "mdpt_set_class_passes": (ctypes.c_int, [_VP, _I, _I]),
    "mdpt_get_class_passes": (ctypes.c_int, [_VP, _I, ctypes.POINTER(_I)]),
    "mdpt_get_class_f8": (ctypes.c_int, [_VP, _I, ctypes.POINTER(_I)]),
    "mdpt_default_mixed_passes_r05": (None, [_I, ctypes.POINTER(_I)]),
    "mdpt_default_mixed_passes": (None, [ctypes.POINTER(_I)]),
    "mdpt_default_mixed_passes_for": (None, [_I, ctypes.POINTER(_I)]),
    "mdpt_set_weight_rounding_compensation": (ctypes.c_int, [_VP, _I]),
    "mdpt_debug_read": (ctypes.c_int, [_VP, ctypes.c_char_p, _VP, _SZ, _VP, _SZ, _VP]),
    "mdpt_allgather": (ctypes.c_int, [_VP, _VP, _VP, _SZ, _I, _VP]),
}

_LIB = None


def load(auto_build: bool = True) -> ctypes.CDLL:
    global _LIB
    if _LIB is not None:
        return _LIB
    if auto_build and _stale():
        build()
    if not os.path.exists(LIB_PATH):
        raise RuntimeError(f"{LIB_PATH} is missing: run `python -c 'import __graft_entry__ as g; g.build()'` (no CPU fallback exists)")
    lib = ctypes.CDLL(LIB_PATH)
    for name, (res, args) in SYMBOLS.items():
        fn = getattr(lib, name)
        fn.restype = res
        fn.argtypes = args
    if lib.mdpt_abi_version() != ABI_VERSION:
        raise RuntimeError("libmdpt ABI version mismatch")
    _LIB = lib
    return lib


def dtype_code(torch_dtype) -> int:
    import torch
    try:
        return {torch.float32: DTYPE_F32, torch.bfloat16: DTYPE_BF16, torch.float16: DTYPE_F16}[torch_dtype]
    except KeyError:
        raise TypeError(f"libmdpt takes float32, bfloat16 or float16 tensors, not {torch_dtype}") from None


class MdptError(RuntimeError):
    def __init__(self, code: int, message: str):
        super().__init__(f"libmdpt error {code}: {message}")
        self.code = code


def check(lib: ctypes.CDLL, rc: int) -> None:
    if rc != 0:
        raise MdptError(rc, lib.mdpt_last_error().decode("utf-8", "replace"))
```

Before: 777.1 depth-maps/s.

## Add persistent tile-walk GEMM that prefetches next tile's operands during the epilogue

For dense single-pass GEMMs (QKV and generic direct-output modes), the kernel can now launch at most one workgroup per CU and walk several 256x256 tiles in turn. While the current tile's epilogue runs, it issues LDS buffer loads for the first two K-tiles of the next tile, so the next prologue can skip those issues and use adjusted wait counts. This aims to hide prologue load latency and reduce wave-quantization tail effects across many tiles. The cost is a more complex control flow, register pressure from the hook, possible loss of the per-launch XCD tile swizzle locality, and serialization when tile counts are not multiples of the CU count. It is enabled by default (walk_mode=1, grid sized to the CU count).

```diff
diff --git a/include/mdpt.h b/include/mdpt.h
--- a/include/mdpt.h
+++ b/include/mdpt.h
@@ -309,6 +309,7 @@
 
 int mdpt_debug_set_stop(mdpt_handle* h, int32_t block, int32_t step);
 int mdpt_debug_set_ksplit_min(mdpt_handle* h, int32_t min_k_tiles, int32_t four_k_tiles);
+int mdpt_debug_set_gemm_persistent(mdpt_handle* h, int32_t mode, int32_t max_workgroups);
 int mdpt_debug_set_reassemble_overlap(mdpt_handle* h, int32_t on);
 int mdpt_debug_set_wscale_policy(mdpt_handle* h, int32_t all);
 int mdpt_debug_set_side_stream_priority(mdpt_handle* h, int32_t prio);
diff --git a/muggled_dpt_amd/csrc/gemm.hip b/muggled_dpt_amd/csrc/gemm.hip
--- a/muggled_dpt_amd/csrc/gemm.hip
+++ b/muggled_dpt_amd/csrc/gemm.hip
@@ -28,7 +28,11 @@
     const char* prof_name = mdpt_kernel_label<kern>(F8 ? "gemm8_kernel<%d, %d, %d, f8>" : "gemm8_kernel<%d, %d, %d>", AMODE, EKIND, DMODE);
     MdptProfScope prof(prof_name, 2.0 * (p.M_alg > 0 ? p.M_alg : p.M) * p.N * p.K, stream);
     const int ks = (AMODE == MDPT_A_DENSE && EKIND == MDPT_E_GENERIC && DMODE == DM_F32 && p.ksplit > 1) ? p.ksplit : 1;
-    hipLaunchKernelGGL(kern, dim3(tiles, ks), dim3(512), LDS, stream, p);
+    int wgs = tiles;
+    if constexpr (gemm8_walk_kernel<AMODE, EKIND, DMODE, F8>()) {
+        if (p.walk_wgs > 0 && p.walk_wgs < tiles && gemm8_walk_ok(p)) wgs = p.walk_wgs;
+    }
+    hipLaunchKernelGGL(kern, dim3(wgs, ks), dim3(512), LDS, stream, p);
     return (int)hipGetLastError();
 }
 
diff --git a/muggled_dpt_amd/csrc/gemm8.inc b/muggled_dpt_amd/csrc/gemm8.inc
--- a/muggled_dpt_amd/csrc/gemm8.inc
+++ b/muggled_dpt_amd/csrc/gemm8.inc
@@ -234,14 +234,41 @@
     }
 };
 
-template <int AMODE, int EKIND, bool SW, bool RI = false, bool FAST = false, bool F8 = false>
+struct Gemm8Prefetch {
+    static constexpr bool active = true;
+    const GemmParams& p; char* smem; int m0, n0, wave; unsigned fa_voff, fb_voff;
+    __device__ __forceinline__ void operator()() const {
+        if (m0 < 0) return;
+        typedef __attribute__((address_space(3))) void* lds_ptr_t;
+        const int rows_here = p.M - m0 < 256 ? p.M - m0 : 256, cols_here = p.N - n0 < 256 ? p.N - n0 : 256;
+        const __amdgpu_buffer_rsrc_t rs_a = tile_rsrc(p.A_hi + (size_t)m0 * p.lda, (size_t)rows_here * p.lda * 2);
+        const __amdgpu_buffer_rsrc_t rs_w = tile_rsrc(p.W_hi + (size_t)n0 * p.ldw, ((size_t)(cols_here - 1) * p.ldw + p.K) * 2);
+        const int fa_step = 64 * p.lda * 2, fb_step = 64 * p.ldw * 2;
+#pragma unroll
+        for (int kt = 0; kt < 2; ++kt) {
+            char* const buf = smem + kt * (2 * 256 * 128);
+#pragma unroll
+            for (int i = 0; i < 4; ++i) {
+                __builtin_amdgcn_raw_ptr_buffer_load_lds(rs_a, (lds_ptr_t)(buf + (wave + 8 * i) * 1024), 16, fa_voff, kt * 128 + i * fa_step, 0, 0);
+                __builtin_amdgcn_raw_ptr_buffer_load_lds(rs_w, (lds_ptr_t)(buf + 256 * 128 + (wave + 8 * i) * 1024), 16, fb_voff, kt * 128 + i * fb_step, 0, 0);
+            }
+        }
+        PIN();
+    }
+};
+
+template <int AMODE, int EKIND, bool SW, bool RI = false, bool FAST = false, bool F8 = false, bool WALK = false>
 __device__ __forceinline__ void gemm8_body(const GemmParams& p, char* smem, const int dmode, const int m0, const int n0,
-                                           const unsigned long long t_start) {
+                                           const unsigned long long t_start, const bool pref = false, const int next_m0 = -1, const int next_n0 = 0,
+                                           const int rec = -1) {
     static_assert(!RI || SW, "residual-initialised accumulators use the swapped operand order (4 consecutive columns per lane)");
     static_assert(!F8 || (!FAST && !RI && MDPT_HAVE_F8), "fp8 cross terms: state-machine stager, fp16 build");
     static_assert(!FAST || AMODE == MDPT_A_DENSE, "the stateless staging is for dense rows");
+    static_assert(!WALK || FAST, "the tile walk prefetches through the stateless staging");
     constexpr int A_BYTES = 256 * 128, BUF = 2 * A_BYTES;
-    const int tid = threadIdx.x, lane = tid & 63;
+    int tid_o = threadIdx.x;
+    if constexpr (WALK) asm volatile("" : "+v"(tid_o));
+    const int tid = tid_o, lane = tid & 63;
     const int wave = __builtin_amdgcn_readfirstlane(tid >> 6);
     const int grp = wave >> 2, wc = wave & 3;
     unsigned long long t_first = 0, t_loop = 0;
@@ -361,10 +388,13 @@
     const int T8 = F8 ? ktiles_f8(p, p.K) : 0, T8a = F8 ? p.K / 128 : 0;
     char* const bufE = smem;
     char* const bufO = smem + BUF;
-    ISSUE_A(0, bufE, 0);
-    ISSUE_B(0, bufE, 0);
-    ISSUE_B(1, bufE, 0);
-    ISSUE_A(1, bufE, 0);
+    const bool entered = WALK && pref;
+    if (!entered) {
+        ISSUE_A(0, bufE, 0);
+        ISSUE_B(0, bufE, 0);
+        ISSUE_B(1, bufE, 0);
+        ISSUE_A(1, bufE, 0);
+    }
     if constexpr (RI) {
         constexpr unsigned OOB = 0xFFFFFFF0u;
         typedef __attribute__((ext_vector_type(4))) int i32x4;
@@ -390,14 +420,19 @@
             }
         };
         load_quadrant(0, 0);
-        ISSUE_B(0, bufO, 128);
-        ISSUE_A(0, bufO, 128);
-        ISSUE_B(1, bufO, 128);
-        ISSUE_A(1, bufO, 128);
+        if (!entered) {
+            ISSUE_B(0, bufO, 128);
+            ISSUE_A(0, bufO, 128);
+            ISSUE_B(1, bufO, 128);
+            ISSUE_A(1, bufO, 128);
+        }
         load_quadrant(0, 1);
         load_quadrant(1, 1);
         load_quadrant(1, 0);
-        WAIT_VM(40);
+        if (entered) WAIT_VM(32);
+        else WAIT_VM(40);
+    } else if (entered) {
+        WAIT_VM(16);
     } else {
         ISSUE_B(0, bufO, 128);
         ISSUE_A(0, bufO, 128);
@@ -424,7 +459,7 @@
                                                                                                               \
         LOAD_B(fb0, 0, 0); PIN(); LOAD_A(0, 0); PIN();                                                                \
         WAIT_LGKM(8); BAR(); WAIT_LGKM(0); PIN();                                                                     \
-        if (FIRST_) { ACC_READY(0, 0, 32); SCALE_Q(0, 0); PIN(); }                     \
+        if (FIRST_) { if (entered) ACC_READY(0, 0, 24); else ACC_READY(0, 0, 32); SCALE_Q(0, 0); PIN(); }  \
         MQ(0, 0, fb0); BAR();                                                                                     \
                                                                                                               \
         LOAD_B(fb1, 1, 0); PIN();                                                                                     \
@@ -501,11 +536,15 @@
 #undef MFMA_Q8_ONE
 #endif
     if (p.dbg_times) t_loop = memtime_now();
+    const auto hook = [&] {
+        if constexpr (WALK) return Gemm8Prefetch{p, smem, next_m0, next_n0, wave, fa_voff, fb_voff};
+        else return NoPrefetch{};
+    }();
     if constexpr (SW) {
         if (EKIND == MDPT_E_SWQKV) {
             if (dmode == DM_F32) {
-                if (HAVE_IMGB && p.bias_img_stride) epilogue_direct<DM_F32, false, MDPT_ACT_NONE, HAVE_IMGB>(p, acc, m0, n0, grp, wc, lane);
-                else epilogue_direct<DM_F32, false, MDPT_ACT_NONE>(p, acc, m0, n0, grp, wc, lane);
+                if (HAVE_IMGB && p.bias_img_stride) epilogue_direct<DM_F32, false, MDPT_ACT_NONE, HAVE_IMGB>(p, acc, m0, n0, grp, wc, lane, hook);
+                else epilogue_direct<DM_F32, false, MDPT_ACT_NONE>(p, acc, m0, n0, grp, wc, lane, hook);
             } else if (HAVE_IMGB && p.bias_img_stride) {
                 if (p.q_lo) epilogue_swin_qk<true, HAVE_IMGB>(p, acc, m0, n0, grp, wc, lane);
                 else epilogue_swin_qk<false, HAVE_IMGB>(p, acc, m0, n0, grp, wc, lane);
@@ -516,37 +555,37 @@
             }
         } else if (EKIND == MDPT_E_QKV) {
             if (HAVE_IMGB && p.bias_img_stride) {
-                if (p.q_lo) epilogue_direct<DM_QK, true, MDPT_ACT_NONE, HAVE_IMGB>(p, acc, m0, n0, grp, wc, lane);
-                else epilogue_direct<DM_QK, false, MDPT_ACT_NONE, HAVE_IMGB>(p, acc, m0, n0, grp, wc, lane);
-            } else if (p.q_lo) epilogue_direct<DM_QK, true, MDPT_ACT_NONE>(p, acc, m0, n0, grp, wc, lane);
-            else epilogue_direct<DM_QK, false, MDPT_ACT_NONE>(p, acc, m0, n0, grp, wc, lane);
+                if (p.q_lo) epilogue_direct<DM_QK, true, MDPT_ACT_NONE, HAVE_IMGB>(p, acc, m0, n0, grp, wc, lane, hook);
+                else epilogue_direct<DM_QK, false, MDPT_ACT_NONE, HAVE_IMGB>(p, acc, m0, n0, grp, wc, lane, hook);
+            } else if (p.q_lo) epilogue_direct<DM_QK, true, MDPT_ACT_NONE>(p, acc, m0, n0, grp, wc, lane, hook);
+            else epilogue_direct<DM_QK, false, MDPT_ACT_NONE>(p, acc, m0, n0, grp, wc, lane, hook);
         } else if (HAVE_IMGB && dmode == DM_BF16 && p.bias_img_stride) {
             if (p.act == MDPT_ACT_GELU) {
-                if (p.out_lo) epilogue_direct<DM_BF16, true, MDPT_ACT_GELU, HAVE_IMGB>(p, acc, m0, n0, grp, wc, lane);
-                else epilogue_direct<DM_BF16, false, MDPT_ACT_GELU, HAVE_IMGB>(p, acc, m0, n0, grp, wc, lane);
+                if (p.out_lo) epilogue_direct<DM_BF16, true, MDPT_ACT_GELU, HAVE_IMGB>(p, acc, m0, n0, grp, wc, lane, hook);
+                else epilogue_direct<DM_BF16, false, MDPT_ACT_GELU, HAVE_IMGB>(p, acc, m0, n0, grp, wc, lane, hook);
             } else {
-                if (p.out_lo) epilogue_direct<DM_BF16, true, MDPT_ACT_NONE, HAVE_IMGB>(p, acc, m0, n0, grp, wc, lane);
-                else epilogue_direct<DM_BF16, false, MDPT_ACT_NONE, HAVE_IMGB>(p, acc, m0, n0, grp, wc, lane);
+                if (p.out_lo) epilogue_direct<DM_BF16, true, MDPT_ACT_NONE, HAVE_IMGB>(p, acc, m0, n0, grp, wc, lane, hook);
+                else epilogue_direct<DM_BF16, false, MDPT_ACT_NONE, HAVE_IMGB>(p, acc, m0, n0, grp, wc, lane, hook);
             }
         } else if (dmode == DM_BF16) {
             const int sel = (p.out_lo ? 3 : 0) + (p.act == MDPT_ACT_GELU ? 2 : (p.act == MDPT_ACT_RELU || p.relu_bf16) ? 1 : 0);
             switch (sel) {
-                case 0: epilogue_direct<DM_BF16, false, MDPT_ACT_NONE>(p, acc, m0, n0, grp, wc, lane); break;
-                case 1: epilogue_direct<DM_BF16, false, MDPT_ACT_RELU>(p, acc, m0, n0, grp, wc, lane); break;
-                case 2: epilogue_direct<DM_BF16, false, MDPT_ACT_GELU>(p, acc, m0, n0, grp, wc, lane); break;
-                case 3: epilogue_direct<DM_BF16, true, MDPT_ACT_NONE>(p, acc, m0, n0, grp, wc, lane); break;
-                case 4: epilogue_direct<DM_BF16, true, MDPT_ACT_RELU>(p, acc, m0, n0, grp, wc, lane); break;
-                default: epilogue_direct<DM_BF16, true, MDPT_ACT_GELU>(p, acc, m0, n0, grp, wc, lane); break;
+                case 0: epilogue_direct<DM_BF16, false, MDPT_ACT_NONE>(p, acc, m0, n0, grp, wc, lane, hook); break;
+                case 1: epilogue_direct<DM_BF16, false, MDPT_ACT_RELU>(p, acc, m0, n0, grp, wc, lane, hook); break;
+                case 2: epilogue_direct<DM_BF16, false, MDPT_ACT_GELU>(p, acc, m0, n0, grp, wc, lane, hook); break;
+                case 3: epilogue_direct<DM_BF16, true, MDPT_ACT_NONE>(p, acc, m0, n0, grp, wc, lane, hook); break;
+                case 4: epilogue_direct<DM_BF16, true, MDPT_ACT_RELU>(p, acc, m0, n0, grp, wc, lane, hook); break;
+                default: epilogue_direct<DM_BF16, true, MDPT_ACT_GELU>(p, acc, m0, n0, grp, wc, lane, hook); break;
             }
         } else if (dmode == DM_F32 || dmode == DM_RINIT) {
-            if (HAVE_IMGB && p.bias_img_stride) epilogue_direct<DM_F32, false, MDPT_ACT_NONE, HAVE_IMGB>(p, acc, m0, n0, grp, wc, lane);
-            else epilogue_direct<DM_F32, false, MDPT_ACT_NONE>(p, acc, m0, n0, grp, wc, lane);
+            if (HAVE_IMGB && p.bias_img_stride) epilogue_direct<DM_F32, false, MDPT_ACT_NONE, HAVE_IMGB>(p, acc, m0, n0, grp, wc, lane, hook);
+            else epilogue_direct<DM_F32, false, MDPT_ACT_NONE>(p, acc, m0, n0, grp, wc, lane, hook);
         } else {
-            epilogue_direct<DM_RESID, false, MDPT_ACT_NONE>(p, acc, m0, n0, grp, wc, lane);
+            if constexpr (!WALK) epilogue_direct<DM_RESID, false, MDPT_ACT_NONE>(p, acc, m0, n0, grp, wc, lane);
         }
         if (p.dbg_times && tid == 0) {
             const unsigned long long t_issued = memtime_now();
-            stamp_record(p.dbg_times, t_start, t_first, t_loop, STAMP_HW_ID, t_issued);
+            stamp_record(p.dbg_times, t_start, t_first, t_loop, STAMP_HW_ID, t_issued, rec);
         }
         return;
     }
@@ -558,14 +597,14 @@
             } else if (p.vt_lo) epilogue_swin_vt<true>(p, acc, m0, n0, grp, wc, lane);
             else epilogue_swin_vt<false>(p, acc, m0, n0, grp, wc, lane);
         } else if (HAVE_IMGB && p.bias_img_stride) {
-            if (p.vt_lo) epilogue_direct_vt<true, HAVE_IMGB>(p, acc, m0, n0, grp, wc, lane);
-            else epilogue_direct_vt<false, HAVE_IMGB>(p, acc, m0, n0, grp, wc, lane);
+            if (p.vt_lo) epilogue_direct_vt<true, HAVE_IMGB>(p, acc, m0, n0, grp, wc, lane, hook);
+            else epilogue_direct_vt<false, HAVE_IMGB>(p, acc, m0, n0, grp, wc, lane, hook);
         } else if (p.vt_lo) {
-            epilogue_direct_vt<true>(p, acc, m0, n0, grp, wc, lane);
+            epilogue_direct_vt<true>(p, acc, m0, n0, grp, wc, lane, hook);
         } else {
-            epilogue_direct_vt<false>(p, acc, m0, n0, grp, wc, lane);
-        }
-        if (p.dbg_times && tid == 0) stamp_record(p.dbg_times, t_start, t_first, t_loop, STAMP_NO_ID);
+            epilogue_direct_vt<false>(p, acc, m0, n0, grp, wc, lane, hook);
+        }
+        if (p.dbg_times && tid == 0) stamp_record(p.dbg_times, t_start, t_first, t_loop, STAMP_NO_ID, 0, rec);
         return;
     }
     __syncthreads();
@@ -601,11 +640,46 @@
     return DM_NONE;
 }
 
+template <int AMODE, int EKIND, int DMODE, bool F8>
+__host__ __device__ constexpr bool gemm8_walk_kernel() {
+#ifdef MDPT_GEMM8_NO_FAST
+    return false;
+#else
+    return AMODE == MDPT_A_DENSE && !F8 && (EKIND == MDPT_E_QKV || (EKIND == MDPT_E_GENERIC && DMODE != DM_NONE && DMODE != DM_RESID));
+#endif
+}
+__host__ __device__ inline bool gemm8_walk_ok(const GemmParams& p) {
+    if (p.npass != 1 || p.ksplit > 1 || p.f8) return false;
+    if (p.ekind == MDPT_E_QKV)
+        return (2 * p.F) % 256 == 0 && p.N % 256 == 0 && (size_t)p.M * p.F * 2 < 0xFFFFFFF0ull && (size_t)(p.M / p.npad) * p.F * p.npadv * 2 < 0xFFFFFFF0ull;
+    return true;
+}
+
 template <int AMODE, int EKIND, int DMODE, bool F8 = false>
 __global__ __launch_bounds__(512, 1) void gemm8_kernel(const GemmParams p) {
     extern __shared__ __attribute__((aligned(16))) char smem[];
     unsigned long long t_start = 0;
     if (p.dbg_times) t_start = memtime_now();
+    if constexpr (gemm8_walk_kernel<AMODE, EKIND, DMODE, F8>()) {
+        const int tiles_n = (p.N + 255) / 256, tiles = tiles_n * ((p.M + 255) / 256), G = gridDim.x;
+        if (G < tiles) {
+            bool pref = false;
+            for (int tile = blockIdx.x; tile < tiles; tile += G) {
+                int m0, n0, m1 = -1, n1 = 0;
+                tile_coords_at(tiles, tile, tiles_n, 256, 256, m0, n0);
+                if (tile + G < tiles) tile_coords_at(tiles, tile + G, tiles_n, 256, 256, m1, n1);
+                if constexpr (EKIND == MDPT_E_QKV) {
+                    if (n0 < 2 * p.F) gemm8_body<AMODE, EKIND, true, false, true, false, true>(p, smem, DM_QK, m0, n0, t_start, pref, m1, n1, tile);
+                    else gemm8_body<AMODE, EKIND, false, false, true, false, true>(p, smem, DM_VT, m0, n0, t_start, pref, m1, n1, tile);
+                } else {
+                    gemm8_body<AMODE, EKIND, true, DMODE == DM_RINIT, true, false, true>(p, smem, DMODE, m0, n0, t_start, pref, m1, n1, tile);
+                }
+                pref = m1 >= 0;
+                if (p.dbg_times) t_start = memtime_now();
+            }
+            return;
+        }
+    }
     int m0, n0;
     tile_coords((p.N + 255) / 256, 256, 256, m0, n0);
     if constexpr (EKIND == MDPT_E_SWQKV) {
diff --git a/muggled_dpt_amd/csrc/gemm8_epilogues.inc b/muggled_dpt_amd/csrc/gemm8_epilogues.inc
--- a/muggled_dpt_amd/csrc/gemm8_epilogues.inc
+++ b/muggled_dpt_amd/csrc/gemm8_epilogues.inc
@@ -5,8 +5,16 @@
     return __builtin_amdgcn_make_buffer_rsrc(const_cast<void*>(base), 0, (int)(unsigned)(bytes < 0xFFFFFFF0ull ? bytes : 0xFFFFFFF0ull), 0x00020000);
 }
 
-template <int MODE, bool X3, int ACT, bool IMGB = false>
-__device__ __forceinline__ void epilogue_direct(const GemmParams& p, f32x4 (&acc)[2][2][4][2], int m0, int n0, int grp, int wc, int lane) {
+struct NoPrefetch {
+    static constexpr bool active = false;
+    __device__ __forceinline__ void operator()() const {}
+};
+template <class T>
+__device__ __forceinline__ void landed(T& v) { asm volatile("" : "+v"(v)); }
+
+template <int MODE, bool X3, int ACT, bool IMGB = false, class HOOK = NoPrefetch>
+__device__ __forceinline__ void epilogue_direct(const GemmParams& p, f32x4 (&acc)[2][2][4][2], int m0, int n0, int grp, int wc, int lane,
+                                                const HOOK& hook = HOOK()) {
     constexpr unsigned OOB = 0xFFFFFFF0u;
     const int l15 = lane & 15, lh = lane >> 4;
     const int rows_here = p.M - m0 < 256 ? p.M - m0 : 256;
@@ -30,17 +38,33 @@
         const __amdgpu_buffer_rsrc_t rs = tile_rsrc(p.out_f32 + (size_t)m0 * p.ldc, (size_t)rows_here * p.ldc * 4);
         const unsigned row_b = (unsigned)p.ldc * 4u;
         const float inv_s = (MDPT_OP_IS_F16 && p.wscale) ? p.wscale[1] : 1.0f;
-#pragma unroll
-        for (int qn = 0; qn < 2; ++qn) {
-            f32x4 bias[2], biasn[2];
-            unsigned col_off[2];
+        f32x4 bias_h[2][2], biasn_h[2][2];
+        unsigned col_off_h[2][2];
+        auto load_cols = [&](int qn) {
 #pragma unroll
             for (int j = 0; j < 2; ++j) {
                 const int nc = n0 + qn * 128 + wc * 32 + j * 16 + 4 * lh;
-                bias[j] = p.bias ? *(const f32x4*)(bias0 + (nc < p.N ? nc : p.N - 4)) : f32x4{0.0f, 0.0f, 0.0f, 0.0f};
-                if (IMGB) biasn[j] = *(const f32x4*)(bias1 + (nc < p.N ? nc : p.N - 4));
-                col_off[j] = nc < p.N ? (unsigned)nc * 4u : OOB;
-            }
+                bias_h[qn][j] = p.bias ? *(const f32x4*)(bias0 + (nc < p.N ? nc : p.N - 4)) : f32x4{0.0f, 0.0f, 0.0f, 0.0f};
+                if (IMGB) biasn_h[qn][j] = *(const f32x4*)(bias1 + (nc < p.N ? nc : p.N - 4));
+                col_off_h[qn][j] = nc < p.N ? (unsigned)nc * 4u : OOB;
+            }
+        };
+        if constexpr (HOOK::active) {
+            load_cols(0);
+            load_cols(1);
+#pragma unroll
+            for (int q = 0; q < 4; ++q) {
+                landed(bias_h[q >> 1][q & 1]);
+                if (IMGB) landed(biasn_h[q >> 1][q & 1]);
+            }
+            hook();
+        }
+#pragma unroll
+        for (int qn = 0; qn < 2; ++qn) {
+            if constexpr (!HOOK::active) load_cols(qn);
+            const f32x4(&bias)[2] = bias_h[qn];
+            const f32x4(&biasn)[2] = biasn_h[qn];
+            const unsigned(&col_off)[2] = col_off_h[qn];
 #pragma unroll
             for (int qm = 0; qm < 2; ++qm)
 #pragma unroll
@@ -58,6 +82,7 @@
         return;
     }
     if (MODE == DM_RESID) {
+        static_assert(MODE != DM_RESID || !HOOK::active, "the in-place residual form loads between its stores: no place for a hook (gemm8_walk_kernel leaves it out)");
         const __amdgpu_buffer_rsrc_t rs = tile_rsrc(p.out_f32 + (size_t)m0 * p.ldc, (size_t)rows_here * p.ldc * 4);
         const unsigned row_b = (unsigned)p.ldc * 4u;
         f32x4 bias[2][2], gam[2][2];
@@ -151,6 +176,14 @@
             if (MODE == DM_QK && ncol < p.F) gam_q[qn][j] = f32x4{p.qscale, p.qscale, p.qscale, p.qscale};
             else if (MODE == DM_QK) gam_q[qn][j] = f32x4{1.0f, 1.0f, 1.0f, 1.0f};
         }
+    if constexpr (HOOK::active) {
+#pragma unroll
+        for (int q = 0; q < 4; ++q) {
+            landed(bias_q[q >> 1][q & 1]);
+            if (IMGB) landed(biasn_q[q >> 1][q & 1]);
+        }
+        hook();
+    }
 #pragma unroll
     for (int qn = 0; qn < 2; ++qn) {
         const int nq = n0 + qn * 128 + wc * 32;
@@ -448,8 +481,9 @@
                 }
 }
 
-template <bool X3, bool IMGB = false>
-__device__ __forceinline__ void epilogue_direct_vt(const GemmParams& p, f32x4 (&acc)[2][2][4][2], int m0, int n0, int grp, int wc, int lane) {
+template <bool X3, bool IMGB = false, class HOOK = NoPrefetch>
+__device__ __forceinline__ void epilogue_direct_vt(const GemmParams& p, f32x4 (&acc)[2][2][4][2], int m0, int n0, int grp, int wc, int lane,
+                                                   const HOOK& hook = HOOK()) {
     constexpr unsigned OOB = 0xFFFFFFF0u;
     const int l15 = lane & 15, lh = lane >> 4;
     const size_t plane = (size_t)(p.M / p.npad) * p.F * p.npadv * 2;
@@ -474,6 +508,14 @@
             bias_q[qn][j] = bias0[n < p.N ? n : p.N - 1];
             if (IMGB) biasn_q[qn][j] = bias1[n < p.N ? n : p.N - 1];
         }
+    if constexpr (HOOK::active) {
+#pragma unroll
+        for (int q = 0; q < 4; ++q) {
+            landed(bias_q[q >> 1][q & 1]);
+            if (IMGB) landed(biasn_q[q >> 1][q & 1]);
+        }
+        hook();
+    }
 #pragma unroll
     for (int qn = 0; qn < 2; ++qn) {
         const int ncol = n0 + qn * 128 + wc * 32 + (lh & 1) * 16 + l15;
diff --git a/muggled_dpt_amd/csrc/gemm_common.inc b/muggled_dpt_amd/csrc/gemm_common.inc
--- a/muggled_dpt_amd/csrc/gemm_common.inc
+++ b/muggled_dpt_amd/csrc/gemm_common.inc
@@ -207,8 +207,10 @@
     }
 };
 
-__device__ __forceinline__ void tile_coords(int tiles_n, int BM, int BN, int& m0, int& n0) {
-    const int nwg = gridDim.x, swz = xcd_tile();
+__device__ __forceinline__ void tile_coords_at(int nwg, int bid, int tiles_n, int BM, int BN, int& m0, int& n0);
+__device__ __forceinline__ void tile_coords(int tiles_n, int BM, int BN, int& m0, int& n0) { tile_coords_at(gridDim.x, blockIdx.x, tiles_n, BM, BN, m0, n0); }
+__device__ __forceinline__ void tile_coords_at(int nwg, int bid, int tiles_n, int BM, int BN, int& m0, int& n0) {
+    const int swz = xcd_tile(nwg, bid);
     if (tiles_n >= 8 && (tiles_n & 3) == 0) {
         const int tiles_m = nwg / tiles_n, per_panel = tiles_m * 4;
         const int panel = swz / per_panel, r = swz - panel * per_panel;
diff --git a/muggled_dpt_amd/csrc/mdpt_debug.cpp b/muggled_dpt_amd/csrc/mdpt_debug.cpp
--- a/muggled_dpt_amd/csrc/mdpt_debug.cpp
+++ b/muggled_dpt_amd/csrc/mdpt_debug.cpp
@@ -47,6 +47,13 @@
     if (!h || min_k_tiles < 2 || four_k_tiles < 4) return fail(MDPT_E_INVALID, "null handle or thresholds below 2 / 4 K tiles");
     h->ks_min_ktiles = min_k_tiles;
     h->ks_big_ktiles = four_k_tiles;
+    return 0;
+}
+
+int mdpt_debug_set_gemm_persistent(mdpt_handle* h, int32_t mode, int32_t max_workgroups) {
+    if (mode < 0 || mode > 1 || max_workgroups < 0) return fail(MDPT_E_INVALID, "gemm persistent: mode 0 or 1, max_workgroups >= 0");
+    if (h) { h->walk_mode = mode; h->walk_max = max_workgroups; }
+    else { g_debug_walk_mode = mode; g_debug_walk_max = max_workgroups; }
     return 0;
 }
 
@@ -123,6 +130,7 @@
     g.act = (tile >> 8) & 3;
     g.out_f32 = (float*)out_f32; g.out_hi = (op_t*)out_bf16; g.ldc = N; g.ldr = N;
     g.dbg_times = (unsigned long long*)dbg_times;
+    g.walk_wgs = debug_walk_wgs();
     if ((tile >> 10) & 1) {
         if (!out_f32 || !out_bf16) return fail(MDPT_E_INVALID, "residual mode needs both output buffers");
         g.bias = (const float*)out_bf16; g.gamma = (const float*)out_bf16 + N; g.resid = (const float*)out_f32; g.out_hi = nullptr;
@@ -225,6 +233,7 @@
     g.head_w = (const float*)f->head_w; g.head_b = (const float*)f->head_b; g.head_sigmoid = f->head_sigmoid; g.head_out = f->head_out;
     g.head_out_dtype = f->head_out_dtype;
     g.ksplit = f->ksplit; g.ks_part = (float*)f->ks_part; g.ks_all = f->ks_all;
+    g.walk_wgs = debug_walk_wgs();
     CHK(OPLG(mdpt_launch_gemm, g, (hipStream_t)stream));
     return 0;
 }
diff --git a/muggled_dpt_amd/csrc/mdpt_internal.h b/muggled_dpt_amd/csrc/mdpt_internal.h
--- a/muggled_dpt_amd/csrc/mdpt_internal.h
+++ b/muggled_dpt_amd/csrc/mdpt_internal.h
@@ -31,6 +31,18 @@
 
 extern thread_local std::string g_err;
 extern int g_debug_f16;
+
+extern int g_debug_walk_mode, g_debug_walk_max;
+inline int device_cu_count() {
+    int dev = 0, cus = 0;
+    if (hipGetDevice(&dev) != hipSuccess || hipDeviceGetAttribute(&cus, hipDeviceAttributeMultiprocessorCount, dev) != hipSuccess) return 0;
+    return cus;
+}
+inline int walk_wgs_for(int mode, int max_wgs, int cus) { return mode == 0 || cus <= 0 ? 0 : (max_wgs > 0 && max_wgs < cus ? max_wgs : cus); }
+inline int debug_walk_wgs() {
+    static const int cus = device_cu_count();
+    return walk_wgs_for(g_debug_walk_mode, g_debug_walk_max, cus);
+}
 
 int fail(int code, const char* fmt, ...);
 
@@ -197,6 +209,12 @@
     }
     void cache_store(int slot, const void* ws, int B, int H, int W) { cache_slot[slot] = CacheSlot{ws, B, H, W, gen, true}; }
     void cache_clear() { cache_slot[0].valid = cache_slot[1].valid = false; }
+    int walk_mode = 1, walk_max = 0;
+    mutable int cu_count = -1;
+    int gemm_walk_wgs() const {
+        if (cu_count < 0) cu_count = device_cu_count();
+        return walk_wgs_for(walk_mode, walk_max, cu_count);
+    }
     int ks_min_ktiles, ks_big_ktiles;
     hipStream_t side_stream, side_cand[4], side_for[4];
     int side_pick[4], side_nfor;
diff --git a/muggled_dpt_amd/csrc/mdpt_inventory.cpp b/muggled_dpt_amd/csrc/mdpt_inventory.cpp
--- a/muggled_dpt_amd/csrc/mdpt_inventory.cpp
+++ b/muggled_dpt_amd/csrc/mdpt_inventory.cpp
@@ -4,6 +4,7 @@
 
 thread_local std::string g_err = "";
 int g_debug_f16 = 0;
+int g_debug_walk_mode = 1, g_debug_walk_max = 0;
 
 int fail(int code, const char* fmt, ...) {
     char buf[1024];
diff --git a/muggled_dpt_amd/csrc/mdpt_kernels.h b/muggled_dpt_amd/csrc/mdpt_kernels.h
--- a/muggled_dpt_amd/csrc/mdpt_kernels.h
+++ b/muggled_dpt_amd/csrc/mdpt_kernels.h
@@ -39,6 +39,7 @@
     const float* pos;
     int d2s_k, d2s_cout;
     const float* head_w; const float* head_b; int head_sigmoid; void* head_out; int head_out_dtype;
+    int walk_wgs;
     int throughput_mode;
     int f8; size_t a8_off;
     const unsigned char* W8; const unsigned char* W8_lo;
diff --git a/muggled_dpt_amd/csrc/mdpt_stages.cpp b/muggled_dpt_amd/csrc/mdpt_stages.cpp
--- a/muggled_dpt_amd/csrc/mdpt_stages.cpp
+++ b/muggled_dpt_amd/csrc/mdpt_stages.cpp
@@ -17,6 +17,7 @@
     g.zero_page = c.h->zero_page;
     g.amode = MDPT_A_DENSE; g.ekind = MDPT_E_GENERIC; g.tile = c.h->gemm_tile;
     g.throughput_mode = c.split ? 1 : 0;
+    g.walk_wgs = c.h->gemm_walk_wgs();
     g.ldc = w.Np; g.ldr = w.Np;
     return g;
 }
diff --git a/muggled_dpt_amd/csrc/mfma_common.inc b/muggled_dpt_amd/csrc/mfma_common.inc
--- a/muggled_dpt_amd/csrc/mfma_common.inc
+++ b/muggled_dpt_amd/csrc/mfma_common.inc
@@ -26,17 +26,17 @@
 #define WAIT_VM(N_) asm volatile("s_waitcnt vmcnt(" #N_ ")" ::: "memory")
 #define WAIT_VM_IMM(N_) asm volatile("s_waitcnt vmcnt(%0)" ::"n"(N_) : "memory")
 
-__device__ __forceinline__ int xcd_tile() {
-    const int nwg = gridDim.x, bid = blockIdx.x;
+__device__ __forceinline__ int xcd_tile(int nwg, int bid) {
     const int xq = nwg >> 3, xr = nwg & 7, xcd = bid & 7;
     return (xcd < xr ? xcd * (xq + 1) : xr * (xq + 1) + (xcd - xr) * xq) + (bid >> 3);
 }
+__device__ __forceinline__ int xcd_tile() { return xcd_tile(gridDim.x, blockIdx.x); }
 
 constexpr int STAMP_HW_ID = -1, STAMP_NO_ID = -2;
 __device__ __forceinline__ void stamp_record(unsigned long long* dbg_times, unsigned long long t_start, unsigned long long t_first, unsigned long long t_loop,
-                                             int xcc_slot, unsigned long long t_issued = 0) {
+                                             int xcc_slot, unsigned long long t_issued = 0, int rec = -1) {
     asm volatile("s_waitcnt vmcnt(0)" ::: "memory");
-    unsigned long long* d = dbg_times + (size_t)blockIdx.x * 6;
+    unsigned long long* d = dbg_times + (size_t)(rec >= 0 ? rec : (int)blockIdx.x) * 6;
     d[0] = t_start; d[1] = t_first; d[2] = t_loop; d[3] = memtime_now();
     if (xcc_slot == STAMP_NO_ID) { d[4] = d[3]; d[5] = 0; return; }
     d[4] = xcc_slot == 4 ? __builtin_amdgcn_s_getreg(20 << 0 | 0 << 6 | 3 << 11) : t_issued;
diff --git a/muggled_dpt_amd/native.py b/muggled_dpt_amd/native.py
--- a/muggled_dpt_amd/native.py
+++ b/muggled_dpt_amd/native.py
@@ -306,6 +306,7 @@
     "mdpt_profile_report": (ctypes.c_int, [ctypes.c_char_p, _SZ]),
     "mdpt_debug_set_stop": (ctypes.c_int, [_VP, _I, _I]),
     "mdpt_debug_set_ksplit_min": (ctypes.c_int, [_VP, _I, _I]),
+    "mdpt_debug_set_gemm_persistent": (ctypes.c_int, [_VP, _I, _I]),
     "mdpt_debug_set_reassemble_overlap": (ctypes.c_int, [_VP, _I]),
     "mdpt_debug_set_wscale_policy": (ctypes.c_int, [_VP, _I]),
     "mdpt_debug_set_side_stream_priority": (ctypes.c_int, [_VP, _I]),
```

After: 776.1 depth-maps/s. No clear change (-0.1%).
